# NilFoundation/crypto3-zk

Hardware: AMD Instinct MI355X
Metric: MSM Mpoints/sec, BLS12-381 G1 Pippenger, 2^20 points per GPU (higher is better)
Workload: dtype u32; 1 GPU; BLS12-381 G1 Pippenger MSM, ONE MSM of 1 x 2^20 random points/scalars, bases resident; points_per_gpu=1048576, parallelism=point-range partition x1 + one all-gather of the 144-B partial sums

## Files before the change

### __graft_entry__.py

```python
import importlib.util
import os
import subprocess
import sys

ROOT = os.path.dirname(os.path.abspath(__file__))


def _load_pkg():
    if "crypto3_zk_amd" in sys.modules:
        return sys.modules["crypto3_zk_amd"]
    pkg_dir = os.path.join(ROOT, "crypto3-zk_amd")
    spec = importlib.util.spec_from_file_location("crypto3_zk_amd", os.path.join(pkg_dir, "__init__.py"),
                                                  submodule_search_locations=[pkg_dir])
    mod = importlib.util.module_from_spec(spec)
    sys.modules["crypto3_zk_amd"] = mod
    spec.loader.exec_module(mod)
    return mod


def build() -> None:
    env = dict(os.environ)
    subprocess.check_call(["make", "-C", os.path.join(ROOT, "crypto3-zk_amd"), "-j4", "all"], env=env)
    subprocess.check_call(["make", "-C", os.path.join(ROOT, "oracle"), "liboracle.so"], env=env)
    subprocess.check_call(["make", "-j2", "-C", os.path.join(ROOT, "tests", "cpp")], env=env)
    subprocess.check_call(["make", "-C", os.path.join(ROOT, "tests", "cpp"), "-f", "merkle.mk"], env=env)
    subprocess.check_call(["make", "-C", os.path.join(ROOT, "tests", "cpp"), "-f", "pow.mk"], env=env)
    subprocess.check_call(["make", "-j2", "-C", os.path.join(ROOT, "tests", "cpp"), "-f", "pasta.mk"], env=env)
    subprocess.check_call(["make", "-C", os.path.join(ROOT, "tests", "cpp"), "-f", "ipa.mk"], env=env)
    zk = _load_pkg()
    zk.load_library()


def smoke() -> None:
    import numpy as np

    sys.path.insert(0, os.path.join(ROOT, "oracle"))
    import cport as cp
    import pyoracle as po

    zk = _load_pkg()
    ctx = zk.Context(0)
    n = 5000
    ks = cp.random_fr(0, 1, n)
    bases = ctx.bases_from_scalars(zk.BLS12_381, zk.G1, ks)
    pts, inf = bases.download()
    exp_pts, _ = cp.batch_mul(0, 1, ks)
    assert (pts == exp_pts).all(), "device fixed-base multiples differ from the oracle"
    sc = cp.random_fr(0, 2, n)
    aff, is_inf = ctx.msm_affine(bases, sc)
    exp, einf = cp.msm(0, 1, pts, sc, chunks=2)
    assert is_inf == einf and (aff == exp).all(), "MSM differs from the oracle"
    grp = zk.DeviceGroup([0, 0])
    gb = grp.upload_bases(zk.BLS12_381, zk.G1, pts)
    gaff, ginf = grp.msm_affine(gb, sc)
    assert ginf == einf and (gaff == exp).all(), "device-group MSM differs from the oracle"
    gb.free()
    grp.close()
    k2 = cp.random_fr(0, 4, 300)
    b2 = ctx.bases_from_scalars(zk.BLS12_381, zk.G2, k2)
    p2, _ = b2.download()
    s2 = cp.random_fr(0, 5, 300)
    aff2, inf2 = ctx.msm_affine(b2, s2)
    exp2, einf2 = cp.msm(0, 2, p2, s2, chunks=2)
    assert inf2 == einf2 and (aff2 == exp2).all(), "G2 MSM differs from the oracle"
    b2.free()
    log_m = 12
    w = np.array(po.to_limbs(po.BLS12_381.root_of_unity(log_m), 4), dtype=np.uint64)
    a = cp.random_fr(0, 3, 2 << log_m).reshape(2, 1 << log_m, 4)
    got = ctx.ntt(zk.BLS12_381, a, log_m, w)
    assert (got == cp.ntt(0, a, log_m, w)).all(), "NTT differs from the oracle"
    assert (ctx.ntt(zk.BLS12_381, got, log_m, w, inverse=True) == a).all()
    bases.free()
    M, nin = 1024, 10
    g16 = cp.Groth16(0, M, nin, seed=3)
    kind, m = cp.domain_choice(M + nin + 1, 32)
    wd = np.array(po.to_limbs(po.BLS12_381.root_of_unity((M + nin).bit_length()), 4), dtype=np.uint64)
    gen = np.array(po.to_limbs(po.BLS12_381.fr_generator, 4), dtype=np.uint64)
    g16.set_domain(kind, m, wd)
    r1cs = ctx.upload_r1cs(zk.BLS12_381, g16.M, g16.n, g16.N, g16.csr(0), g16.csr(1), g16.csr(2))
    assert (r1cs.kind, r1cs.m) == (kind, m) == (2, 1040), "the constraint system's domain is not the reference's choice"
    z = np.concatenate([np.array([[1, 0, 0, 0]], dtype=np.uint64), g16.assignment()])
    assert (ctx.groth16_witness_h(r1cs, z, wd, gen) == g16.witness_map(wd, gen)).all(), "witness map over the step domain differs from the oracle"
    r1cs.free()
    import hashlib
    state = hashlib.sha256(b"zkhip smoke").digest()
    k = next(k for k in range(1 << 20)
             if int.from_bytes(hashlib.sha256(hashlib.sha256(state + (12345 + k).to_bytes(4, "big")).digest()).digest()[28:], "big") & 0xFFF == 0)
    assert ctx.pow_grind(state, 12345, 0xFFF) == (12345 + k, k + 1), "the device's proof of work is not the first accepted nonce"
    ctx.close()
    print("smoke ok: G1 MSM n=5000 (one context and a device group of two), G2 MSM n=300, NTT 2^12 x 2 and the witness map over a step radix-2 domain bit-exact against the oracle; proof of work (12 bits) = the reference loop's nonce")


if __name__ == "__main__":
    build()
    if len(sys.argv) > 1 and sys.argv[1] == "smoke":
        smoke()
```

### crypto3-zk_amd/csrc/ctx.hpp

```cpp
#pragma once
#include <hip/hip_runtime.h>

#include <algorithm>
#include <cassert>
#include <cstdint>
#include <cstdio>
#include <cstring>
#include <map>
#include <memory>
#include <mutex>
#include <string>
#include <type_traits>
#include <unordered_map>
#include <unordered_set>
#include <utility>
#include <vector>

#include "../../include/zkhip.h"
#include "options.hpp"
#include "table_cache.hpp"
#include "zk_defs.hpp"

#define ZK_HIP_CHECK(ctx, expr)                                                                  \
    do {                                                                                         \
        hipError_t e__ = (expr);                                                                 \
        if (e__ != hipSuccess) {                                                                 \
            (ctx)->last_error = std::string(#expr) + ": " + hipGetErrorString(e__);              \
            return e__ == hipErrorOutOfMemory ? ZKHIP_ERR_OOM : ZKHIP_ERR_HIP;                   \
        }                                                                                        \
    } while (0)

#define ZK_TRY(expr)              \
    do {                          \
        int rc__ = (expr);        \
        if (rc__ != 0) return rc__; \
    } while (0)

inline bool zk_curve_known(int curve) { return curve >= zkhip::CURVE_BLS12_381 && curve <= zkhip::CURVE_VESTA; }
inline bool zk_curve_pairing(int curve) { return curve == zkhip::CURVE_BLS12_381 || curve == zkhip::CURVE_BN254; }
inline bool zk_group_known(int group) { return group == zkhip::GROUP_G1 || group == zkhip::GROUP_G2; }
inline bool zk_curve_group_known(int curve, int group) { return zk_curve_known(curve) && (group == zkhip::GROUP_G1 || (group == zkhip::GROUP_G2 && zk_curve_pairing(curve))); }
#define ZK_ARGS(ctx, curve) if (!(ctx) || !zk_curve_known(curve)) return ZKHIP_ERR_INVALID
#define ZK_ARGS_PAIRING(ctx, curve) if (!(ctx) || !zk_curve_pairing(curve)) return ZKHIP_ERR_INVALID
#define ZK_ENTER(ctx) ZK_HIP_CHECK(ctx, hipSetDevice((ctx)->device))
inline bool zk_any_null(const void *const *p, size_t count) {
    return std::any_of(p, p + count, [](const void *q) { return !q; });
}

inline dim3 grid_1d(size_t count, unsigned threads = 256) {
    const size_t groups = (count + threads - 1) / threads;
    assert(groups < ((size_t)1 << 31));
    return dim3((unsigned)groups);
}

static constexpr int ZK_MSM_MAX_C = 21;

enum : uint32_t { ZK_STATUS_GATHER_RANGE = 1u, ZK_STATUS_MSM_PLAN_OVERFLOW = 2u, ZK_STATUS_LOOKUP_NOT_IN_TABLE = 4u, ZK_STATUS_LOOKUP_SORT_OVERFLOW = 8u };

struct zkhip_ctx;

struct DevBuf {
    uint32_t *p = nullptr;
    DevBuf() = default;
    DevBuf(const DevBuf &) = delete;
    DevBuf &operator=(const DevBuf &) = delete;
    DevBuf(DevBuf &&o) noexcept : p(o.p) { o.p = nullptr; }
    DevBuf &operator=(DevBuf &&o) noexcept {
        if (this != &o) {
            reset();
            p = o.p;
            o.p = nullptr;
        }
        return *this;
    }
    ~DevBuf() { reset(); }
    void reset() {
        if (p) (void)hipFree(p);
        p = nullptr;
    }
    int alloc(zkhip_ctx *ctx, size_t bytes);
    operator uint32_t *() const { return p; }
    template <class T>
    T *as() const { return reinterpret_cast<T *>(p); }
};
template <bool Pinned = false>
struct GrowBuf {
    void *p = nullptr;
    size_t cap = 0;
    GrowBuf() = default;
    GrowBuf(const GrowBuf &) = delete;
    GrowBuf &operator=(const GrowBuf &) = delete;
    GrowBuf(GrowBuf &&o) noexcept : p(o.p), cap(o.cap) { o.p = nullptr, o.cap = 0; }
    ~GrowBuf() { reset(); }
    void reset() {
        if (p) (void)(Pinned ? hipHostFree(p) : hipFree(p));
        p = nullptr;
        cap = 0;
    }
    int reserve(zkhip_ctx *ctx, size_t bytes, size_t slack = 0);
    template <class T>
    T *as() const { return static_cast<T *>(p); }
};
struct ZkHipDelete {
    void operator()(hipEvent_t e) const { (void)hipEventDestroy(e); }
    void operator()(hipStream_t s) const { (void)hipStreamDestroy(s); }
    void operator()(hipGraphExec_t g) const { (void)hipGraphExecDestroy(g); }
};
using EventOwner = std::unique_ptr<std::remove_pointer_t<hipEvent_t>, ZkHipDelete>;
using StreamOwner = std::unique_ptr<std::remove_pointer_t<hipStream_t>, ZkHipDelete>;
using GraphExecOwner = std::unique_ptr<std::remove_pointer_t<hipGraphExec_t>, ZkHipDelete>;
inline hipError_t zk_event_create(EventOwner &e, unsigned flags = hipEventDefault) {
    hipEvent_t raw = nullptr;
    const hipError_t rc = hipEventCreateWithFlags(&raw, flags);
    e.reset(raw);
    return rc;
}

struct zkhip_bases {
    int curve, group;
    size_t n;
    size_t stride_u32;
    DevBuf d;
    int c_tab = 0, ntab = 1;
    int win_rank = 0, win_world = 1;
    int nslots = 1;
    bool tables() const { return c_tab > 0; }
    int local_windows() const { return win_rank < ntab ? (ntab - win_rank + win_world - 1) / win_world : 0; }
    int slot_of_local(int lw) const { return lw + (win_rank != 0 ? 1 : 0); }
};

struct ZkEventPair {
    EventOwner a, b;
};

struct ZkProfile {
    bool on = false;
    bool last_recorded = false;
    std::string filter;
    std::vector<std::pair<std::string, ZkEventPair>> pending;
    std::vector<ZkEventPair> pool;
    std::map<std::string, std::pair<double, uint64_t>> acc;
};

static constexpr int NTT_MAX_PASSES = 32;
struct NttTables {
    int curve;
    size_t log_m;
    int inverse;
    bool has_coset;
    int smax, tile_log;
    uint64_t omega[4], coset[4];
    int lo_bits;
    DevBuf d_tw[NTT_MAX_PASSES];
    DevBuf d_stage[NTT_MAX_PASSES];
    DevBuf d_prepost;
    DevBuf d_lo, d_hi;
    DevBuf d_clo, d_chi;
    DevBuf d_scale;
    DevBuf d_base;
};
struct NttExtTables {
    int curve;
    size_t log_m, log_k;
    uint64_t omega_big[4];
    DevBuf d_pre;
};
struct DomTables {
    int curve, kind;
    size_t m, n0, n1;
    uint64_t omega[4], shift[4], coset[4];
    bool has_coset;
    DevBuf d_T;
    DevBuf d_Tinv;
    DevBuf d_consts;
    DevBuf d_zinv;
    size_t nz = 1;
    uint64_t w0[4], w1[4];
    uint64_t coset1[4];
};

struct ZkGraph {
    GraphExecOwner exec;
    uint64_t ws_epoch = 0;
    DevBuf d_ptrs;
};

struct zkhip_ctx {
    int device = 0;
    hipStream_t stream = nullptr;
    StreamOwner own_stream;
    EventOwner order_event;
    std::string last_error;
    std::multimap<size_t, void *> alloc_free;
    std::unordered_map<void *, size_t> alloc_live;
    size_t alloc_cached_bytes = 0, opt_alloc_cache_bytes = (size_t)16 << 30;
    std::mutex alloc_mutex;
    DevBuf d_status;
    GrowBuf<> ws;
    size_t ws_off = 0, ws_floor = 0;
    std::unordered_set<const void *> lds_configured;
    std::unordered_map<std::string, ZkGraph> graphs;
    std::unordered_map<std::string, int> graph_seen;
    uint64_t ws_epoch = 0;
    bool capturing = false;
    void *batch_dptrs_override = nullptr;
    int opt_msm_graphs = 0;
    GrowBuf<> msm_host_buf;
    int opt_msm_window_bits = 0;
    int opt_msm_sets = 0;
    int opt_msm_sort_tile_log = 14;
    int opt_ec_ntt_table_lanes = 0;
    int opt_msm_share_sort = 1;
    int opt_msm_tail_quads = 1;
    int opt_msm_tail_fold = 16;
    int opt_msm_tail_fold_g2 = 1;
    int opt_msm_fold_run = 0;
    int opt_msm_segment_log = -1;
    int opt_ntt_radix_log = 8;
    int opt_ntt_tile_log = 3;
    int opt_poly_coset_extend = 1;
    int opt_ntt_pair = 1;
    int opt_msm_precompute = 1;
    int opt_msm_shard_rank = 0, opt_msm_shard_world = 1;
    int opt_stream_priority = 0;
    int opt_msm_precompute_min = 32;
    ZkProfile prof;
    TableCache<NttTables> ntt_tables{24};
    TableCache<NttExtTables> ntt_ext_tables{16};
    TableCache<DomTables> dom_tables{8};
    GrowBuf<> dom_ws;

    zkhip_ctx() = default;
    ~zkhip_ctx();

    int ws_reserve(size_t bytes) {
        if (bytes <= ws.cap) return 0;
        if (capturing) {
            last_error = "workspace growth during graph capture";
            return ZKHIP_ERR_HIP;
        }
        ++ws_epoch;
        return ws.reserve(this, bytes, (bytes >> 3) + (1 << 20));
    }
    void ws_reset() { ws_off = ws_floor; }
    static size_t ws_round(size_t bytes) { return (bytes + 255) & ~(size_t)255; }
    int stream_drain() {
        ZK_HIP_CHECK(this, hipStreamSynchronize(stream));
        return 0;
    }

    void prof_begin(const char *name) {
        prof.last_recorded = false;
        if (!prof.on) return;
        if (!prof.filter.empty() && strncmp(name, prof.filter.c_str(), prof.filter.size()) != 0) return;
        prof.last_recorded = true;
        ZkEventPair ev;
        if (!prof.pool.empty()) {
            ev = std::move(prof.pool.back());
            prof.pool.pop_back();
        } else {
            (void)zk_event_create(ev.a);
            (void)zk_event_create(ev.b);
        }
        (void)hipEventRecord(ev.a.get(), stream);
        prof.pending.emplace_back(name, std::move(ev));
    }
    void prof_end() {
        if (!prof.on || !prof.last_recorded) return;
        (void)hipEventRecord(prof.pending.back().second.b.get(), stream);
    }
    void prof_collect() {
        if (prof.pending.empty()) return;
        (void)hipStreamSynchronize(stream);
        for (auto &p : prof.pending) {
            float ms = 0;
            (void)hipEventElapsedTime(&ms, p.second.a.get(), p.second.b.get());
            auto &a = prof.acc[p.first];
            a.first += ms;
            a.second += 1;
            prof.pool.push_back(std::move(p.second));
        }
        prof.pending.clear();
    }
};

inline int DevBuf::alloc(zkhip_ctx *ctx, size_t bytes) {
    reset();
    const hipError_t e = hipMalloc((void **)&p, bytes);
    if (e == hipSuccess) return 0;
    (void)hipGetLastError();
    ctx->last_error = "hipMalloc(" + std::to_string(bytes) + " bytes): " + hipGetErrorString(e);
    return ZKHIP_ERR_OOM;
}
template <bool Pinned>
int GrowBuf<Pinned>::reserve(zkhip_ctx *ctx, size_t bytes, size_t slack) {
    if (bytes <= cap) return 0;
    if (p) ZK_HIP_CHECK(ctx, hipStreamSynchronize(ctx->stream));
    reset();
    const hipError_t e = Pinned ? hipHostMalloc(&p, bytes + slack, hipHostMallocPortable) : hipMalloc(&p, bytes + slack);
    if (e != hipSuccess) {
        (void)hipGetLastError();
        p = nullptr;
        ctx->last_error = std::string(Pinned ? "hipHostMalloc(" : "hipMalloc(") + std::to_string(bytes + slack) + " bytes): " + hipGetErrorString(e);
        return ZKHIP_ERR_OOM;
    }
    cap = bytes + slack;
    return 0;
}

struct WsCount {
    size_t bytes = 0;
    template <class T>
    void take(T *&, size_t count) { bytes += zkhip_ctx::ws_round(count * sizeof(T)); }
};
struct WsBump {
    zkhip_ctx *ctx;
    template <class T>
    void take(T *&p, size_t count) {
        p = reinterpret_cast<T *>(ctx->ws.as<char>() + ctx->ws_off);
        ctx->ws_off += zkhip_ctx::ws_round(count * sizeof(T));
    }
};
template <class T>
struct WsOne {
    size_t count;
    T *p;
    template <class Arena>
    void layout(Arena &a) { a.take(p, count); }
};
template <class Layout>
size_t ws_bytes(Layout &l) {
    WsCount a;
    l.layout(a);
    return a.bytes;
}
template <class Layout>
int ws_place(zkhip_ctx *ctx, Layout &l, size_t above = 0) {
    const size_t end = ctx->ws_floor + ws_bytes(l);
    ZK_TRY(ctx->ws_reserve(end + above));
    ctx->ws_reset();
    WsBump a{ctx};
    l.layout(a);
    if (ctx->ws_off > end || end + above > ctx->ws.cap) {
        ctx->last_error = "workspace layout took " + std::to_string(ctx->ws_off - ctx->ws_floor) + " bytes of " + std::to_string(end - ctx->ws_floor) + " reserved";
        return ZKHIP_ERR_RANGE;
    }
    return 0;
}

inline int ws_upload(zkhip_ctx *ctx, void *d_dst, const void *src, size_t bytes) {
    if (ctx->capturing) {
        ctx->last_error = "host table upload during graph capture";
        return ZKHIP_ERR_HIP;
    }
    ZK_HIP_CHECK(ctx, hipMemcpyAsync(d_dst, src, bytes, hipMemcpyHostToDevice, ctx->stream));
    return 0;
}

#define ZK_MAX_LDS(ctx, kernel, bytes)                                                                                              \
    do {                                                                                                                            \
        const void *fn__ = reinterpret_cast<const void *>(&kernel);                                                                 \
        if ((ctx)->lds_configured.insert(fn__).second)                                                                              \
            ZK_HIP_CHECK(ctx, hipFuncSetAttribute(fn__, hipFuncAttributeMaxDynamicSharedMemorySize, (int)(bytes)));                 \
    } while (0)

#define ZK_LAUNCH(ctx, name, kernel, grid, block, lds, ...)                        \
    do {                                                                           \
        (ctx)->prof_begin(name);                                                   \
        hipLaunchKernelGGL(kernel, grid, block, lds, (ctx)->stream, __VA_ARGS__);  \
        (ctx)->prof_end();                                                         \
        ZK_HIP_CHECK(ctx, hipGetLastError());                                      \
    } while (0)

int zk_msm_run(zkhip_ctx *ctx, const zkhip_bases *bases, size_t offset, size_t n, const uint32_t *d_scalars, uint32_t *d_out_jac);
int zk_msm_run_batch(zkhip_ctx *ctx, size_t count, const zkhip_bases *const *bases, const size_t *offsets, const size_t *ns,
                     const uint32_t *const *d_scalars, uint32_t *const *d_outs);
size_t zk_coord_limbs64(int curve, int group);
int zk_bases_to_mont(zkhip_ctx *ctx, zkhip_bases *b, const uint32_t *d_canonical, const uint8_t *d_inf);
size_t zk_point_words(int curve, int group);
int zk_msm_auto_window(size_t n);
int zk_scalar_bits(int curve);
int zk_bases_decompress(zkhip_ctx *ctx, zkhip_bases *b, const uint8_t *d_octets, uint32_t *d_err);
void zk_graphs_clear(zkhip_ctx *ctx);
int zk_bases_precompute(zkhip_ctx *ctx, zkhip_bases *b);
int zk_bases_from_mont(zkhip_ctx *ctx, const zkhip_bases *b, size_t offset, size_t n, uint32_t *d_out, uint8_t *d_inf);
int zk_bases_mul(zkhip_ctx *ctx, zkhip_bases *b, const uint32_t *d_base_canonical , const uint32_t *d_scalars);
int zk_jac_sum(zkhip_ctx *ctx, int curve, int group, const uint32_t *d_pts, size_t count, uint32_t *d_out);
int zk_jac_to_affine(zkhip_ctx *ctx, int curve, int group, const uint32_t *d_jac, uint32_t *d_aff, uint8_t *d_inf);
int zk_ntt_run(zkhip_ctx *ctx, int curve, uint32_t *d_data, size_t log_m, size_t batch, const uint64_t *omega, int inverse,
               const uint64_t *coset);
int zk_ntt_extend(zkhip_ctx *ctx, int curve, uint32_t *d_coeffs, size_t log_m, size_t batch, const uint64_t *omega, uint32_t *d_out, size_t log_k,
                  const uint64_t *omega_big);
int zk_msm_host_reserve(zkhip_ctx *ctx, size_t n);
```

### crypto3-zk_amd/csrc/hosttest.hip

```cpp
#include <cstring>
#include <vector>

#define ZK_NOINLINE_MUL 1
#include "arith_ops.h"
#include "msm_recode.hpp"
#include "pow.hpp"
#include "sha256.hpp"

using namespace zkhip;
using namespace zkhip::arith;

#define FIELD_SWITCH(field, ...)                             \
    switch (field) {                                         \
        case 0: { typedef bls_fq F; __VA_ARGS__; } break;    \
        case 1: { typedef bls_fr F; __VA_ARGS__; } break;    \
        case 2: { typedef bn_fq F; __VA_ARGS__; } break;     \
        case 3: { typedef bn_fr F; __VA_ARGS__; } break;     \
        case 4: { typedef bls_fq2 F; __VA_ARGS__; } break;   \
        case 5: { typedef bn_fq2 F; __VA_ARGS__; } break;    \
        case 6: { typedef bls_fqu F; __VA_ARGS__; } break;   \
        case 7: { typedef bn_fqu F; __VA_ARGS__; } break;    \
        case 8: { typedef bls_fru F; __VA_ARGS__; } break;   \
        case 9: { typedef bn_fru F; __VA_ARGS__; } break;    \
        case 10: { typedef bls_fqu2 F; __VA_ARGS__; } break; \
        case 11: { typedef bn_fqu2 F; __VA_ARGS__; } break;  \
        case 12: { typedef pallas_fq F; __VA_ARGS__; } break; \
        case 13: { typedef pallas_fr F; __VA_ARGS__; } break; \
        case 14: { typedef vesta_fq F; __VA_ARGS__; } break;  \
        case 15: { typedef vesta_fr F; __VA_ARGS__; } break;  \
        case 16: { typedef pallas_fqu F; __VA_ARGS__; } break; \
        case 17: { typedef vesta_fqu F; __VA_ARGS__; } break; \
        case 18: { typedef pallas_fru F; __VA_ARGS__; } break; \
        case 19: { typedef vesta_fru F; __VA_ARGS__; } break; \
        default: return -1;                                  \
    }

extern "C" {

int zkt_field_op(int field, int op, const uint32_t *a, const uint32_t *b, uint32_t *out) {
    if (!field_op_valid(op)) return -1;
    FIELD_SWITCH(field, field_op<F>(op, a, b, out); return 0);
    return -1;
}

int zkt_fu_raw(int type, int op, size_t n, const uint32_t *a, const uint32_t *b, const uint32_t *c, const uint32_t *d, uint32_t *out) {
#define FU_RAW(U)                                                                                                       \
    {                                                                                                                   \
        if (!fu_raw_valid<U>(op)) return -1;                                                                            \
        for (size_t i = 0; i < n; ++i) fu_raw_one<U>(op, a + i * U::L, b + i * U::L, c + i * U::L, d + i * U::L, out + i * U::L); \
        return 0;                                                                                                       \
    }
    switch (type) {
        case 6: FU_RAW(BlsFqU)
        case 7: FU_RAW(BnFqU)
        case 8: FU_RAW(BlsFrU)
        case 9: FU_RAW(BnFrU)
        case 16: FU_RAW(PallasFqU)
        case 17: FU_RAW(VestaFqU)
        case 18: FU_RAW(PallasFrU)
        case 19: FU_RAW(VestaFrU)
        default: return -1;
    }
#undef FU_RAW
}

int zkt_point_chain(int field, const uint32_t *pts, const uint8_t *inf, const uint8_t *neg, size_t n, int mode, uint32_t k,
                    uint32_t *out, uint8_t *out_inf) {
    if (field == 1 || field == 3 || field == 8 || field == 9 || field == 13 || field == 15 || field == 18 || field == 19) return -1;
    FIELD_SWITCH(field, point_chain<F>(pts, inf, neg, n, mode, k, out, out_inf); return 0);
    return -1;
}

static int recode_windows(const uint32_t *scalar, MsmWindows win, int32_t *digits) {
    uint32_t carry = 0;
    for (int w = 0; w < win.W; ++w) {
        uint32_t d = msm_recode(scalar, win.off(w), win.width(w), carry);
        if (d == DIG_NONE) digits[w] = 0;
        else {
            int32_t mag = (int32_t)(d & 0x7FFFFFFFu) + 1;
            digits[w] = (d >> 31) ? -mag : mag;
        }
    }
    return (int)carry;
}

int zkt_recode(const uint32_t *scalar, int c, int W, int32_t *digits) { return recode_windows(scalar, msm_make_windows(c * W, W), digits); }

int zkt_recode_folded(int curve, const uint32_t *scalar, int c, int32_t *digits) {
    uint32_t s[8];
    bool flip = false;
    if (fr_sat_dispatch(curve, [&](auto fr) -> int {
            flip = msm_fold_scalar<typename decltype(fr)::type>(scalar, s);
            return 0;
        }) != 0)
        return -1;
    const int tb = curve == CURVE_BN254 ? 254 : 255, W = msm_windows(tb, c);
    if (recode_windows(s, msm_make_windows(tb, W), digits) != 0) return -1;
    if (flip)
        for (int w = 0; w < W; ++w) digits[w] = -digits[w];
    return W;
}

int zkt_sha256_elements(const uint64_t *elems, size_t n, uint8_t *digest) {
    if (!elems || !digest || n == 0) return -1;
    sha256::hash_elements(elems, n, digest);
    return 0;
}

int zkt_merkle_tree(const uint64_t *leaves, size_t n_leaves, size_t per_leaf, uint8_t *digests) {
    if (!leaves || !digests || n_leaves == 0 || (n_leaves & (n_leaves - 1)) || per_leaf == 0) return -1;
    for (size_t x = 0; x < n_leaves; ++x) sha256::hash_elements(leaves + 4 * x * per_leaf, per_leaf, digests + 32 * x);
    uint8_t *level = digests;
    for (size_t n = n_leaves / 2; n >= 1; n /= 2) {
        uint8_t *up = level + 64 * n;
        for (size_t j = 0; j < n; ++j) sha256::hash_node(level + 64 * j, level + 64 * j + 32, up + 32 * j);
        level = up;
    }
    return 0;
}

uint32_t zkt_pow_candidate(const uint8_t *state, uint32_t nonce) { return pow::candidate(pow::prepare(state), nonce); }

int zkt_pow_grind_cpu(const uint8_t *state, uint32_t start, uint32_t mask, uint64_t max_tries, uint32_t *nonce, uint64_t *tried) {
    if (!state || !nonce || !tried || max_tries > ((uint64_t)1 << 32)) return -1;
    const uint64_t total = max_tries ? max_tries : (uint64_t)1 << 32, k = pow::first_hit(pow::prepare(state), start, mask, total);
    *tried = k < total ? k + 1 : total;
    if (k == total) return 1;
    *nonce = start + (uint32_t)k;
    return 0;
}

int zkt_sha256_bytes(const uint8_t *msg, size_t len, uint8_t *digest) {
    if (!digest || (!msg && len)) return -1;
    pow::hash_bytes(msg, len, digest);
    return 0;
}

}
```

### crypto3-zk_amd/csrc/msm_core.hpp

```cpp
#pragma once
#include <algorithm>
#include <string>
#include <type_traits>
#include <vector>

#ifndef ZK_NOINLINE_MUL2
#define ZK_NOINLINE_MUL2 1
#endif
#include "ctx.hpp"
#include "curve.hpp"
#include "msm_ops.hpp"
#include "msm_recode.hpp"
#include "msm_bucket_acc.hpp"
#include "fu_pair.hpp"
#include "fu_quad.hpp"

namespace {

using namespace zkhip;

constexpr uint32_t MSM_LARGE_BUCKET = 128;
constexpr uint32_t MSM_LARGE_CHUNK = 4096;
#ifndef MSM_G1_THREADS
#define MSM_G1_THREADS 64
#endif
#ifndef MSM_G2_THREADS
#define MSM_G2_THREADS 256
#endif
#ifndef MSM_G2_WAVES
#define MSM_G2_WAVES 2
#endif

template <uint32_t THREADS>
ZK_D void block_inclusive_scan(uint32_t *scratch) {
    const uint32_t t = threadIdx.x;
    __syncthreads();
    for (uint32_t d = 1; d < THREADS; d <<= 1) {
        uint32_t x = t >= d ? scratch[t - d] : 0;
        __syncthreads();
        scratch[t] += x;
        __syncthreads();
    }
}

__global__ __launch_bounds__(256) void msm_scan_local(const uint32_t *__restrict__ hist, uint32_t count, uint32_t *__restrict__ offs,
                                                      uint32_t *__restrict__ block_sums) {
    __shared__ uint32_t part[256];
    const uint32_t t = threadIdx.x, base = blockIdx.x * 1024 + t * 4;
    uint32_t v[4], s = 0;
#pragma unroll
    for (int k = 0; k < 4; ++k) {
        v[k] = base + k < count ? hist[base + k] : 0;
        s += v[k];
    }
    part[t] = s;
    block_inclusive_scan<256>(part);
    uint32_t run = part[t] - s;
#pragma unroll
    for (int k = 0; k < 4; ++k) {
        if (base + k < count) offs[base + k] = run;
        run += v[k];
    }
    if (t == 255) block_sums[blockIdx.x] = part[255];
}

__global__ __launch_bounds__(1024) void msm_scan_top(uint32_t *__restrict__ block_sums, uint32_t nblocks, uint32_t *__restrict__ total) {
    __shared__ uint32_t part[1024];
    const uint32_t t = threadIdx.x;
    const uint32_t per = (nblocks + 1023) / 1024;
    const uint32_t lo = min(nblocks, t * per), hi = min(nblocks, lo + per);
    uint32_t s = 0;
    for (uint32_t i = lo; i < hi; ++i) s += block_sums[i];
    part[t] = s;
    block_inclusive_scan<1024>(part);
    uint32_t run = part[t] - s;
    for (uint32_t i = lo; i < hi; ++i) {
        uint32_t x = block_sums[i];
        block_sums[i] = run;
        run += x;
    }
    if (t == 1023) *total = part[1023];
}

__global__ __launch_bounds__(256) void msm_scan_add(uint32_t *__restrict__ offs, uint32_t count, const uint32_t *__restrict__ block_sums,
                                                    uint32_t *__restrict__ cursor) {
    const uint32_t base = blockIdx.x * 1024 + threadIdx.x * 4;
    const uint32_t add = block_sums[blockIdx.x];
#pragma unroll
    for (int k = 0; k < 4; ++k) {
        if (base + k < count) {
            uint32_t x = offs[base + k] + add;
            offs[base + k] = x;
            cursor[base + k] = x;
        }
    }
}

__global__ __launch_bounds__(1024) void msm_scan_single(const uint32_t *__restrict__ hist, uint32_t count, uint32_t *__restrict__ offs,
                                                        uint32_t *__restrict__ cursor) {
    __shared__ uint32_t part[1024];
    __shared__ uint32_t carry;
    const uint32_t t = threadIdx.x;
    if (t == 0) carry = 0;
    __syncthreads();
    for (uint32_t base = 0; base < count; base += 1024) {
        const uint32_t v = base + t < count ? hist[base + t] : 0;
        part[t] = v;
        block_inclusive_scan<1024>(part);
        const uint32_t excl = carry + part[t] - v;
        if (base + t < count) {
            offs[base + t] = excl;
            if (cursor != offs) cursor[base + t] = excl;
        }
        __syncthreads();
        if (t == 1023) carry += part[1023];
        __syncthreads();
    }
    if (t == 0) offs[count] = carry;
}
constexpr uint32_t MSM_SCAN_SINGLE_MAX = 1u << 16;

inline int msm_scan(zkhip_ctx *ctx, const char *name, const uint32_t *hist, uint32_t count, uint32_t *offs, uint32_t *bsums) {
    if (count <= MSM_SCAN_SINGLE_MAX) {
        ZK_LAUNCH(ctx, name, msm_scan_single, dim3(1), dim3(1024), 0, hist, count, offs, offs);
        return 0;
    }
    const uint32_t nblk = (count + 1023) / 1024;
    ZK_LAUNCH(ctx, name, msm_scan_local, dim3(nblk), dim3(256), 0, hist, count, offs, bsums);
    ZK_LAUNCH(ctx, name, msm_scan_top, dim3(1), dim3(1024), 0, bsums, nblk, offs + count);
    ZK_LAUNCH(ctx, name, msm_scan_add, dim3(nblk), dim3(256), 0, offs, count, bsums, offs);
    return 0;
}

template <class FR>
__global__ __launch_bounds__(256) void msm_digits_only(const uint32_t *__restrict__ scalars, uint32_t n, MsmWindows win, uint32_t wrank,
                                                       uint32_t wworld, uint32_t *__restrict__ dig) {
    uint32_t i = blockIdx.x * blockDim.x + threadIdx.x;
    if (i >= n) return;
    uint32_t s[8];
    const uint32_t flip = msm_fold_scalar<FR>(scalars + (size_t)i * 8, s) ? 0x80000000u : 0u;
    uint32_t carry = 0, next = wrank, lw = 0;
    for (int w = 0; w < win.W; ++w) {
        uint32_t d = msm_recode(s, win.off(w), win.width(w), carry);
        if ((uint32_t)w != next) continue;
        dig[(size_t)lw * n + i] = d == DIG_NONE ? d : d ^ flip;
        next += wworld;
        ++lw;
    }
}

struct SortGeom {
    uint32_t n;
    uint32_t W;
    uint32_t B;
    uint32_t S;
    uint32_t lowb;
    uint32_t nsuper;
    uint32_t tile;
    uint32_t ntile;
    uint32_t slot0;
    uint32_t tables;
    uint32_t bases_n;
    uint32_t base_off;
};
struct SortBig {
    static constexpr uint32_t TILE = 16384, THREADS = 1024;
};
struct SortSmall {
    static constexpr uint32_t TILE = 4096, THREADS = 256;
};
constexpr uint32_t SORT_MAX_LOW = 10;
constexpr uint32_t SORT_MAX_SUPER = 1024;

ZK_D uint32_t sort_key(const SortGeom &g, uint32_t w, uint32_t d) { return (w % g.S) * g.B + (d & 0x7FFFFFFFu); }
ZK_D uint32_t sort_entry(const SortGeom &g, uint32_t w, uint32_t i, uint32_t d) {
    return ((g.tables ? (g.slot0 + w) * g.bases_n : 0u) + g.base_off + i) | (d & 0x80000000u);
}

template <class SZ>
__global__ __launch_bounds__(SZ::THREADS) void msm_sort_hist(const uint32_t *__restrict__ dig, SortGeom g, uint32_t *__restrict__ bh) {
    constexpr uint32_t SORT_TILE = SZ::TILE, SORT_THREADS = SZ::THREADS;
    extern __shared__ uint32_t lh[];
    const uint32_t tile = blockIdx.x, w = blockIdx.y, t = threadIdx.x;
    for (uint32_t k = t; k < g.nsuper; k += SORT_THREADS) lh[k] = 0;
    __syncthreads();
    const uint32_t lo = tile * SORT_TILE, hi = min(g.n, lo + SORT_TILE);
    for (uint32_t i = lo + t; i < hi; i += SORT_THREADS) {
        uint32_t d = dig[(size_t)w * g.n + i];
        if (d != DIG_NONE) atomicAdd(&lh[sort_key(g, w, d) >> g.lowb], 1u);
    }
    __syncthreads();
    const size_t col = (size_t)w * g.ntile + tile, stride = (size_t)g.W * g.ntile;
    for (uint32_t k = t; k < g.nsuper; k += SORT_THREADS) bh[(size_t)k * stride + col] = lh[k];
}

template <uint32_t SORT_THREADS>
ZK_D uint32_t block_excl_scan(uint32_t *v, uint32_t count, uint32_t *scratch ) {
    const uint32_t t = threadIdx.x, per = (count + SORT_THREADS - 1) / SORT_THREADS;
    const uint32_t lo = min(count, t * per), hi = min(count, lo + per);
    uint32_t s = 0;
    for (uint32_t k = lo; k < hi; ++k) s += v[k];
    scratch[t] = s;
    block_inclusive_scan<SORT_THREADS>(scratch);
    const uint32_t total = scratch[SORT_THREADS - 1];
    uint32_t run = scratch[t] - s;
    for (uint32_t k = lo; k < hi; ++k) {
        uint32_t x = v[k];
        v[k] = run;
        run += x;
    }
    __syncthreads();
    return total;
}

template <class SZ>
__global__ __launch_bounds__(SZ::THREADS) void msm_sort_split(const uint32_t *__restrict__ dig, SortGeom g, const uint32_t *__restrict__ bo,
                                                              uint32_t *__restrict__ tmp_idx, uint16_t *__restrict__ tmp_key) {
    constexpr uint32_t SORT_TILE = SZ::TILE, SORT_THREADS = SZ::THREADS;
    extern __shared__ uint32_t sm[];
    uint32_t *loff = sm;
    uint32_t *cur = loff + g.nsuper + 1;
    uint32_t *gbase = cur + g.nsuper;
    uint32_t *scratch = gbase + g.nsuper;
    uint32_t *sidx = scratch + SORT_THREADS;
    uint32_t *skey = sidx + SORT_TILE;
    const uint32_t tile = blockIdx.x, w = blockIdx.y, t = threadIdx.x;
    const size_t col = (size_t)w * g.ntile + tile, stride = (size_t)g.W * g.ntile;
    for (uint32_t k = t; k < g.nsuper; k += SORT_THREADS) {
        loff[k] = 0;
        gbase[k] = bo[(size_t)k * stride + col];
    }
    __syncthreads();
    const uint32_t lo = tile * SORT_TILE, hi = min(g.n, lo + SORT_TILE);
    for (uint32_t i = lo + t; i < hi; i += SORT_THREADS) {
        uint32_t d = dig[(size_t)w * g.n + i];
        if (d != DIG_NONE) atomicAdd(&loff[sort_key(g, w, d) >> g.lowb], 1u);
    }
    __syncthreads();
    const uint32_t total = block_excl_scan<SORT_THREADS>(loff, g.nsuper, scratch);
    if (t == 0) loff[g.nsuper] = total;
    for (uint32_t k = t; k < g.nsuper; k += SORT_THREADS) cur[k] = loff[k];
    __syncthreads();
    for (uint32_t i = lo + t; i < hi; i += SORT_THREADS) {
        uint32_t d = dig[(size_t)w * g.n + i];
        if (d == DIG_NONE) continue;
        const uint32_t key = sort_key(g, w, d);
        const uint32_t r = atomicAdd(&cur[key >> g.lowb], 1u);
        sidx[r] = sort_entry(g, w, i, d);
        skey[r] = key;
    }
    __syncthreads();
    const uint32_t lmask = (1u << g.lowb) - 1;
    for (uint32_t s = t; s < total; s += SORT_THREADS) {
        const uint32_t key = skey[s], bin = key >> g.lowb, pos = gbase[bin] + (s - loff[bin]);
        tmp_idx[pos] = sidx[s];
        tmp_key[pos] = (uint16_t)(key & lmask);
    }
}

constexpr uint32_t SORT_NLOW_MAX = 1u << SORT_MAX_LOW;

template <uint32_t THREADS>
ZK_D void block_scan_counts(const uint32_t *cnt, uint32_t *excl, uint32_t *scratch) {
    constexpr uint32_t CPT = SORT_NLOW_MAX / THREADS;
    const uint32_t t = threadIdx.x;
    uint32_t s = 0;
#pragma unroll
    for (uint32_t k = 0; k < CPT; ++k) s += cnt[t * CPT + k];
    scratch[t] = s;
    block_inclusive_scan<THREADS>(scratch);
    uint32_t run = scratch[t] - s;
#pragma unroll
    for (uint32_t k = 0; k < CPT; ++k) {
        excl[t * CPT + k] = run;
        run += cnt[t * CPT + k];
    }
    __syncthreads();
}

template <class SZ>
__global__ __launch_bounds__(SZ::THREADS) void msm_sort_final(const uint32_t *__restrict__ tmp_idx, const uint16_t *__restrict__ tmp_key, SortGeom g,
                                                              uint32_t nb, const uint32_t *__restrict__ bo, uint32_t *__restrict__ offs,
                                                              uint32_t *__restrict__ idx) {
    constexpr uint32_t SORT_TILE = SZ::TILE, SORT_THREADS = SZ::THREADS;
    __shared__ uint32_t cnt[SORT_NLOW_MAX], cursor[SORT_NLOW_MAX], loff[SORT_NLOW_MAX], cur[SORT_NLOW_MAX], scratch[SORT_THREADS];
    extern __shared__ uint32_t sm[];
    uint32_t *sidx = sm;
    uint16_t *skey = reinterpret_cast<uint16_t *>(sidx + SORT_TILE);
    const uint32_t grp = blockIdx.x, t = threadIdx.x;
    const size_t stride = (size_t)g.W * g.ntile;
    const uint32_t start = bo[(size_t)grp * stride];
    const uint32_t end = bo[(size_t)(grp + 1) * stride];
    const uint32_t nlow = 1u << g.lowb;
    for (uint32_t k = t; k < SORT_NLOW_MAX; k += SORT_THREADS) cnt[k] = 0;
    __syncthreads();
    for (uint32_t k = start + t; k < end; k += SORT_THREADS) atomicAdd(&cnt[tmp_key[k]], 1u);
    __syncthreads();
    block_scan_counts<SORT_THREADS>(cnt, cursor, scratch);
    for (uint32_t k = t; k < nlow; k += SORT_THREADS) {
        const uint32_t bucket = grp * nlow + k;
        cursor[k] += start;
        if (bucket < nb) offs[bucket] = cursor[k];
    }
    if (grp + 1 == g.nsuper && t == 0) offs[nb] = end;
    __syncthreads();
    for (uint32_t c0 = start; c0 < end; c0 += SORT_TILE) {
        const uint32_t c1 = min(end, c0 + SORT_TILE);
        for (uint32_t k = t; k < SORT_NLOW_MAX; k += SORT_THREADS) cnt[k] = 0;
        __syncthreads();
        for (uint32_t k = c0 + t; k < c1; k += SORT_THREADS) atomicAdd(&cnt[tmp_key[k]], 1u);
        __syncthreads();
        block_scan_counts<SORT_THREADS>(cnt, loff, scratch);
        for (uint32_t k = t; k < SORT_NLOW_MAX; k += SORT_THREADS) cur[k] = loff[k];
        __syncthreads();
        for (uint32_t k = c0 + t; k < c1; k += SORT_THREADS) {
            const uint32_t key = tmp_key[k];
            const uint32_t r = atomicAdd(&cur[key], 1u);
            sidx[r] = tmp_idx[k];
            skey[r] = (uint16_t)key;
        }
        __syncthreads();
        for (uint32_t s = t; s < c1 - c0; s += SORT_THREADS) {
            const uint32_t key = skey[s];
            idx[cursor[key] + (s - loff[key])] = sidx[s];
        }
        __syncthreads();
        for (uint32_t k = t; k < SORT_NLOW_MAX; k += SORT_THREADS) cursor[k] += cnt[k];
        __syncthreads();
    }
}

constexpr uint32_t SIZE_BINS = MSM_LARGE_BUCKET + 2;

ZK_D uint32_t size_bin(uint32_t size, uint32_t large) {
    if (size == 0 || size > large) return SIZE_BINS - 1;
    return size > MSM_LARGE_BUCKET ? 0 : 1 + MSM_LARGE_BUCKET - size;
}

__global__ __launch_bounds__(256) void msm_size_hist(const uint32_t *__restrict__ offs, uint32_t nbuckets, uint32_t nblocks,
                                                     uint32_t large, uint32_t *__restrict__ bh) {
    __shared__ uint32_t lh[SIZE_BINS];
    const uint32_t t = threadIdx.x;
    if (t < SIZE_BINS) lh[t] = 0;
    __syncthreads();
    for (uint32_t g = blockIdx.x * 1024 + t; g < min(nbuckets, (blockIdx.x + 1) * 1024); g += 256)
        atomicAdd(&lh[size_bin(offs[g + 1] - offs[g], large)], 1u);
    __syncthreads();
    if (t < SIZE_BINS) bh[(size_t)t * nblocks + blockIdx.x] = lh[t];
}

__global__ __launch_bounds__(256) void msm_size_scatter(const uint32_t *__restrict__ offs, uint32_t nbuckets, uint32_t nblocks,
                                                        uint32_t large, const uint32_t *__restrict__ bo, uint32_t *__restrict__ order) {
    __shared__ uint32_t cur[SIZE_BINS];
    const uint32_t t = threadIdx.x;
    if (t < SIZE_BINS) cur[t] = bo[(size_t)t * nblocks + blockIdx.x];
    __syncthreads();
    for (uint32_t g = blockIdx.x * 1024 + t; g < min(nbuckets, (blockIdx.x + 1) * 1024); g += 256)
        order[atomicAdd(&cur[size_bin(offs[g + 1] - offs[g], large)], 1u)] = g;
}

__global__ __launch_bounds__(256) void msm_plan_large(const uint32_t *__restrict__ offs, uint32_t nbuckets, uint32_t *__restrict__ plan,
                                                      uint32_t *__restrict__ tasks, uint32_t *__restrict__ large, uint32_t task_cap,
                                                      uint32_t large_cap, uint32_t thresh, uint32_t *__restrict__ status) {
    uint32_t g = blockIdx.x * blockDim.x + threadIdx.x;
    if (g >= nbuckets) return;
    uint32_t lo = offs[g], hi = offs[g + 1], size = hi - lo;
    if (size <= thresh) return;
    uint32_t nt = (size + MSM_LARGE_CHUNK - 1) / MSM_LARGE_CHUNK;
    uint32_t first = atomicAdd(&plan[0], nt);
    uint32_t slot = atomicAdd(&plan[1], 1u);
    if (first + nt > task_cap || slot >= large_cap) {
        atomicOr(status, ZK_STATUS_MSM_PLAN_OVERFLOW);
        return;
    }
    for (uint32_t t = 0; t < nt; ++t) {
        tasks[3 * (first + t)] = g;
        tasks[3 * (first + t) + 1] = lo + t * MSM_LARGE_CHUNK;
        tasks[3 * (first + t) + 2] = min(hi, lo + (t + 1) * MSM_LARGE_CHUNK);
    }
    large[3 * slot] = g;
    large[3 * slot + 1] = first;
    large[3 * slot + 2] = nt;
}

template <class F, int LPB>
__global__ __launch_bounds__(128) void msm_bucket_large(const uint32_t *__restrict__ bases, const uint32_t *__restrict__ idx,
                                                        const uint32_t *__restrict__ plan, const uint32_t *__restrict__ tasks,
                                                        uint32_t *__restrict__ partials) {
    constexpr int NL = FieldOps<F>::WORDS;
    extern __shared__ __attribute__((aligned(16))) uint32_t lds[];
    const uint32_t ntasks = plan[0];
    for (uint32_t task = blockIdx.x; task < ntasks; task += gridDim.x) {
        const uint32_t lo = tasks[3 * task + 1], hi = tasks[3 * task + 2], t = threadIdx.x / LPB;
        XYZZ<F> acc = XYZZ<F>::infinity();
        for (uint32_t k = lo + t; k < hi; k += blockDim.x / LPB) {
            uint32_t e = idx[k];
            Affine<F> p = affine_load<F>(bases + (size_t)(e & 0x7FFFFFFFu) * (2 * NL));
            acc = xyzz_madd(acc, p, (e >> 31) != 0);
        }
        xyzz_store<F>(lds + (size_t)t * (4 * NL), acc);
        __syncthreads();
        for (uint32_t d = blockDim.x / LPB / 2; d >= 1; d >>= 1) {
            if (t < d) {
                acc = xyzz_add(xyzz_load<F>(lds + (size_t)t * (4 * NL)), xyzz_load<F>(lds + (size_t)(t + d) * (4 * NL)));
                xyzz_store<F>(lds + (size_t)t * (4 * NL), acc);
            }
            __syncthreads();
        }
        if (t == 0) xyzz_store<F>(partials + (size_t)task * (4 * NL), acc);
        __syncthreads();
    }
}

template <class F, int LPB>
__global__ __launch_bounds__(64) void msm_large_combine(const uint32_t *__restrict__ plan, const uint32_t *__restrict__ large,
                                                        const uint32_t *__restrict__ partials, uint32_t *__restrict__ buckets) {
    constexpr int NL = FieldOps<F>::WORDS;
    extern __shared__ __attribute__((aligned(16))) uint32_t lds[];
    const uint32_t nlarge = plan[1], t = threadIdx.x / LPB;
    for (uint32_t j = blockIdx.x; j < nlarge; j += gridDim.x) {
        const uint32_t g = large[3 * j], first = large[3 * j + 1], nt = large[3 * j + 2];
        XYZZ<F> acc = XYZZ<F>::infinity();
        for (uint32_t k = t; k < nt; k += 64 / LPB) acc = xyzz_add(acc, xyzz_load<F>(partials + (size_t)(first + k) * (4 * NL)));
        if (nt > 1) {
            xyzz_store<F>(lds + (size_t)t * (4 * NL), acc);
            __syncthreads();
            for (uint32_t d = 32 / LPB; d >= 1; d >>= 1) {
                if (t < d && t + d < nt) {
                    acc = xyzz_add(xyzz_load<F>(lds + (size_t)t * (4 * NL)), xyzz_load<F>(lds + (size_t)(t + d) * (4 * NL)));
                    xyzz_store<F>(lds + (size_t)t * (4 * NL), acc);
                }
                __syncthreads();
            }
        }
        if (t == 0) xyzz_store<F>(buckets + (size_t)g * (4 * NL), acc);
        __syncthreads();
    }
}

template <class F, int LPB>
__global__ __launch_bounds__(256) void msm_bucket_merge(uint32_t *__restrict__ buckets, uint32_t B, uint32_t q, uint32_t cur) {
    constexpr int NL = FieldOps<F>::WORDS;
    uint32_t g = (blockIdx.x * blockDim.x + threadIdx.x) / LPB;
    if (g >= q * B) return;
    const uint32_t s = g / B;
    uint32_t *dst = buckets + (size_t)g * (4 * NL);
    XYZZ<F> acc = xyzz_load<F>(dst);
    for (uint32_t k = 1; k < 4; ++k)
        if (s + k * q < cur) acc = xyzz_add(acc, xyzz_load<F>(buckets + ((size_t)g + (size_t)k * q * B) * (4 * NL)));
    xyzz_store<F>(dst, acc);
}

constexpr int MSM_TAIL_THREADS = 256;

template <class F>
ZK_D XYZZ<F> block_tree_sum(uint32_t *lds, XYZZ<F> acc, uint32_t t, uint32_t nthreads) {
    constexpr int NL = FieldOps<F>::WORDS;
    xyzz_store<F>(lds + (size_t)t * (4 * NL), acc);
    __syncthreads();
    for (uint32_t d = nthreads / 2; d >= 1; d >>= 1) {
        if (t < d) {
            acc = xyzz_add(xyzz_load<F>(lds + (size_t)t * (4 * NL)), xyzz_load<F>(lds + (size_t)(t + d) * (4 * NL)));
            xyzz_store<F>(lds + (size_t)t * (4 * NL), acc);
        }
        __syncthreads();
    }
    return acc;
}

template <class F, int LPB>
#ifndef ZK_TAIL_WAVES
#define ZK_TAIL_WAVES 2
#endif
__global__ __launch_bounds__(MSM_TAIL_THREADS, ZK_TAIL_WAVES) void msm_bucket_red(const uint32_t *__restrict__ buckets, uint32_t B, uint32_t L, uint32_t nseg,
                                                                   uint32_t nblk, uint32_t *__restrict__ partial) {
    constexpr int NL = FieldOps<F>::WORDS;
    extern __shared__ __attribute__((aligned(16))) uint32_t lds[];
    constexpr uint32_t SLOTS = MSM_TAIL_THREADS / LPB;
    const uint32_t t = threadIdx.x / LPB, w = blockIdx.x / nblk, seg = (blockIdx.x % nblk) * SLOTS + t;
    XYZZ<F> sum = XYZZ<F>::infinity();
    if (seg < nseg) {
        const uint32_t *base = buckets + ((size_t)w * B + (size_t)seg * L) * (4 * NL);
        if (L == 1) {
            sum = xyzz_mul_small(xyzz_load<F>(base), seg + 1);
        } else {
            XYZZ<F> run = XYZZ<F>::infinity();
            for (int b = (int)L - 1; b >= 0; --b) {
                run = xyzz_add(run, xyzz_load<F>(base + (size_t)b * (4 * NL)));
                sum = xyzz_add(sum, run);
            }
            if (seg != 0) sum = xyzz_add(sum, xyzz_mul_small(run, seg * L));
        }
    }
    sum = block_tree_sum<F>(lds, sum, t, SLOTS);
    if (t == 0) xyzz_store<F>(partial + (size_t)blockIdx.x * (4 * NL), sum);
}

template <class F, int LPB>
__global__ __launch_bounds__(256) void msm_window_sum(const uint32_t *__restrict__ partial, uint32_t nblk, uint32_t *__restrict__ winsum) {
    constexpr int NL = FieldOps<F>::WORDS;
    extern __shared__ __attribute__((aligned(16))) uint32_t lds[];
    const uint32_t w = blockIdx.x, t = threadIdx.x / LPB, slots = blockDim.x / LPB;
    XYZZ<F> acc = XYZZ<F>::infinity();
    for (uint32_t j = t; j < nblk; j += slots) acc = xyzz_add(acc, xyzz_load<F>(partial + ((size_t)w * nblk + j) * (4 * NL)));
    if (nblk > 1) acc = block_tree_sum<F>(lds, acc, t, slots);
    if (t == 0) xyzz_store<F>(winsum + (size_t)w * (4 * NL), acc);
}
inline uint32_t msm_window_threads(uint32_t nblk, int lanes_per_point) { return (size_t)nblk * lanes_per_point > 128 ? 256u : 64u; }

struct MsmFold {
    uint32_t B, C, R, log_c;
    uint32_t run;
    uint32_t m_row, m_col;
};
inline MsmFold msm_fold_geom(const zkhip_ctx *ctx, uint32_t B) {
    MsmFold g;
    int lb = 0;
    while ((1u << lb) < B) ++lb;
    g.B = B;
    g.log_c = (uint32_t)((lb + 1) / 2);
    g.C = 1u << g.log_c;
    g.R = B >> g.log_c;
    g.run = ctx->opt_msm_fold_run > 0 ? (uint32_t)ctx->opt_msm_fold_run : (B >= (1u << 18) ? 8u : 4u);
    g.run = std::max(1u, std::min(g.run, g.R));
    g.m_row = g.C / g.run;
    g.m_col = g.R / g.run;
    return g;
}

template <class FA, int LA, class FT, int LT>
__global__ __launch_bounds__(MSM_TAIL_THREADS, ZK_TAIL_WAVES) void msm_fold(const uint32_t *__restrict__ buckets, MsmFold g, uint32_t *__restrict__ level2) {
    constexpr int NL = FieldOps<FA>::WORDS;
    constexpr uint32_t SA = MSM_TAIL_THREADS / LA, ST = MSM_TAIL_THREADS / LT, PW = 4 * NL;
    extern __shared__ __attribute__((aligned(16))) uint32_t lds[];
    const uint32_t half_wgs = g.B / (SA * g.run);
    const uint32_t w = blockIdx.x / (2 * half_wgs), k = blockIdx.x % (2 * half_wgs);
    const bool col = k >= half_wgs;
    const uint32_t wg = col ? k - half_wgs : k, s = threadIdx.x / LA;
    const uint32_t m = col ? g.m_col : g.m_row, G = SA / m;
    uint32_t first, stride, slot;
    if (!col) {
        first = (wg * G + s / m) * g.C + s % m;
        stride = m;
        slot = s;
    } else {
        const uint32_t j = s / G, ll = s % G;
        first = j * g.C + wg * G + ll;
        stride = m * g.C;
        slot = ll * m + j;
    }
    {
        const uint32_t *src = buckets + ((size_t)w * g.B + first) * PW;
        XYZZ<FA> acc = xyzz_load<FA>(src);
        for (uint32_t i = 1; i < g.run; ++i) acc = xyzz_add(acc, xyzz_load<FA>(src + (size_t)i * stride * PW));
        xyzz_store<FA>(lds + (size_t)slot * PW, acc);
    }
    __syncthreads();
    const uint32_t t = threadIdx.x / LT;
    for (uint32_t half = m / 2; half >= 1; half >>= 1) {
        const uint32_t adds = G * half;
        for (uint32_t idx = t; idx < adds; idx += ST) {
            uint32_t *p = lds + (size_t)((idx / half) * m + idx % half) * PW;
            xyzz_store<FT>(p, xyzz_add(xyzz_load<FT>(p), xyzz_load<FT>(p + (size_t)half * PW)));
        }
        __syncthreads();
    }
    for (uint32_t i = t; i < G; i += ST) {
        const uint32_t o = wg * G + i;
        if (col || o != 0)
            xyzz_store<FT>(level2 + (((size_t)2 * w + (col ? 0 : 1)) * g.C + (col ? o : o - 1)) * PW, xyzz_load<FT>(lds + (size_t)i * m * PW));
    }
}

template <class F>
ZK_D void xyzz_store_canonical_jacobian(uint32_t *dst, const XYZZ<F> &p) {
    constexpr int CW = FieldOps<F>::CANON_WORDS;
    Jacobian<F> j = xyzz_to_jacobian(p);
    FieldOps<F>::to_canonical(dst, j.X);
    FieldOps<F>::to_canonical(dst + CW, j.Y);
    FieldOps<F>::to_canonical(dst + 2 * CW, j.Z);
}

template <class F, int LPB>
__global__ __launch_bounds__(64) void msm_final_fold(const uint32_t *__restrict__ winsum, uint32_t count, uint32_t shift, uint32_t *const *__restrict__ outs,
                                                     uint32_t *__restrict__ out) {
    constexpr int NL = FieldOps<F>::WORDS;
    if (blockIdx.x >= count || threadIdx.x >= LPB) return;
    XYZZ<F> acc = xyzz_load<F>(winsum + ((size_t)2 * blockIdx.x + 1) * (4 * NL));
    if (!acc.is_inf())
        for (uint32_t i = 0; i < shift; ++i) acc = xyzz_dbl(acc);
    acc = xyzz_add(acc, xyzz_load<F>(winsum + (size_t)2 * blockIdx.x * (4 * NL)));
    xyzz_store_canonical_jacobian<F>(outs ? outs[blockIdx.x] : out, acc);
}

template <class F, int LPB>
__global__ __launch_bounds__(64) void msm_final(const uint32_t *__restrict__ winsum, int W, MsmWindows win, uint32_t *__restrict__ out_jac) {
    constexpr int NL = FieldOps<F>::WORDS;
    if (blockIdx.x != 0 || threadIdx.x >= LPB) return;
    XYZZ<F> acc = XYZZ<F>::infinity();
    for (int w = W - 1; w >= 0; --w) {
        if (!acc.is_inf())
            for (int i = 0; i < win.width(w); ++i) acc = xyzz_dbl(acc);
        acc = xyzz_add(acc, xyzz_load<F>(winsum + (size_t)w * (4 * NL)));
    }
    xyzz_store_canonical_jacobian<F>(out_jac, acc);
}

template <class F>
__global__ __launch_bounds__(256) void bases_to_mont(const uint32_t *__restrict__ canon, const uint8_t *__restrict__ inf, uint32_t n,
                                                     uint32_t *__restrict__ pts) {
    typedef FieldOps<F> O;
    uint32_t i = blockIdx.x * blockDim.x + threadIdx.x;
    if (i >= n) return;
    const uint32_t *c = canon + (size_t)i * (2 * O::CANON_WORDS);
    Affine<F> a;
    if (inf != nullptr && inf[i]) a = Affine<F>::infinity();
    else a = {O::from_canonical(c), O::from_canonical(c + O::CANON_WORDS)};
    affine_store<F>(pts + (size_t)i * (2 * O::WORDS), a);
}

template <class F>
__global__ __launch_bounds__(256) void bases_from_mont(const uint32_t *__restrict__ pts, uint32_t n, uint32_t *__restrict__ out,
                                                       uint8_t *__restrict__ inf) {
    typedef FieldOps<F> O;
    uint32_t i = blockIdx.x * blockDim.x + threadIdx.x;
    if (i >= n) return;
    Affine<F> a = affine_load<F>(pts + (size_t)i * (2 * O::WORDS));
    inf[i] = a.is_inf() ? 1 : 0;
    uint32_t *o = out + (size_t)i * (2 * O::CANON_WORDS);
    O::to_canonical(o, a.x);
    O::to_canonical(o + O::CANON_WORDS, a.y);
}

template <class F>
__global__ __launch_bounds__(64) void bases_mul(uint32_t *__restrict__ pts, const uint32_t *__restrict__ base_canonical,
                                                const uint32_t *__restrict__ scalars, uint32_t n) {
    constexpr int NL = FieldOps<F>::WORDS;
    uint32_t i = blockIdx.x * blockDim.x + threadIdx.x;
    if (i >= n) return;
    Affine<F> g = {FieldOps<F>::from_canonical(base_canonical), FieldOps<F>::from_canonical(base_canonical + FieldOps<F>::CANON_WORDS)};
    const uint32_t *s = scalars + (size_t)i * 8;
    XYZZ<F> acc = XYZZ<F>::infinity();
    for (int b = 255; b >= 0; --b) {
        acc = xyzz_dbl(acc);
        if ((s[b >> 5] >> (b & 31)) & 1) acc = xyzz_madd(acc, g);
    }
    affine_store<F>(pts + (size_t)i * (2 * NL), xyzz_to_affine(acc));
}

constexpr int FIXED_WBITS = 8, FIXED_NW = 32, FIXED_ROW = 1 << FIXED_WBITS;
template <class F>
__global__ __launch_bounds__(64) void bases_fixed_table(const uint32_t *__restrict__ base_canonical, uint32_t *__restrict__ tab, uint32_t *__restrict__ tmp) {
    typedef FieldOps<F> O;
    constexpr int NL = O::WORDS;
    const uint32_t w = blockIdx.x * blockDim.x + threadIdx.x;
    if (w >= FIXED_NW) return;
    Affine<F> g = {O::from_canonical(base_canonical), O::from_canonical(base_canonical + O::CANON_WORDS)};
    XYZZ<F> P = XYZZ<F>::from_affine(g);
    for (uint32_t k = 0; k < w * FIXED_WBITS; ++k) P = xyzz_dbl(P);
    uint32_t *mine = tmp + (size_t)w * FIXED_ROW * (5 * NL);
    XYZZ<F> acc = P;
    F pre = F::one();
    for (uint32_t d = 1; d < FIXED_ROW; ++d) {
        if (d > 1) acc = xyzz_add(acc, P);
        uint32_t *slot = mine + (size_t)d * (5 * NL);
        xyzz_store<F>(slot, acc);
        pre = O::mul(pre, O::mul(acc.ZZ, acc.ZZZ));
        O::store(slot + 4 * NL, pre);
    }
    F inv = O::inv(pre);
    for (uint32_t d = FIXED_ROW; d-- > 1;) {
        const uint32_t *slot = mine + (size_t)d * (5 * NL);
        XYZZ<F> q = xyzz_load<F>(slot);
        F before = d > 1 ? O::load(mine + (size_t)(d - 1) * (5 * NL) + 4 * NL) : F::one();
        F dinv = O::mul(inv, before);
        inv = O::mul(inv, O::mul(q.ZZ, q.ZZZ));
        Affine<F> a = {O::mul(q.X, O::mul(dinv, q.ZZZ)), O::mul(q.Y, O::mul(dinv, q.ZZ))};
        affine_store<F>(tab + ((size_t)w * FIXED_ROW + d) * (2 * NL), a);
    }
}
constexpr uint32_t FIXED_CHUNK = 8;
template <class F>
__global__ __launch_bounds__(64) void bases_mul_fixed(uint32_t *__restrict__ pts, const uint32_t *__restrict__ tab, const uint32_t *__restrict__ scalars,
                                                      uint32_t n, uint32_t *__restrict__ tmp) {
    typedef FieldOps<F> O;
    constexpr int NL = O::WORDS;
    const uint32_t lo = (blockIdx.x * blockDim.x + threadIdx.x) * FIXED_CHUNK;
    if (lo >= n) return;
    const uint32_t cnt = n - lo < FIXED_CHUNK ? n - lo : FIXED_CHUNK;
    F pre = F::one();
    for (uint32_t k = 0; k < cnt; ++k) {
        const uint32_t *s = scalars + (size_t)(lo + k) * 8;
        XYZZ<F> acc = XYZZ<F>::infinity();
        for (uint32_t w = 0; w < FIXED_NW; ++w) {
            const uint32_t d = (s[w >> 2] >> ((w & 3) * 8)) & 0xFFu;
            if (d) acc = xyzz_madd(acc, affine_load<F>(tab + ((size_t)w * FIXED_ROW + d) * (2 * NL)));
        }
        uint32_t *slot = tmp + (size_t)(lo + k) * (5 * NL);
        xyzz_store<F>(slot, acc);
        if (!acc.is_inf()) pre = O::mul(pre, O::mul(acc.ZZ, acc.ZZZ));
        O::store(slot + 4 * NL, pre);
    }
    F inv = O::inv(pre);
    for (uint32_t k = cnt; k-- > 0;) {
        const uint32_t *slot = tmp + (size_t)(lo + k) * (5 * NL);
        XYZZ<F> q = xyzz_load<F>(slot);
        if (q.is_inf()) {
            affine_store<F>(pts + (size_t)(lo + k) * (2 * NL), Affine<F>::infinity());
            continue;
        }
        F before = k > 0 ? O::load(tmp + (size_t)(lo + k - 1) * (5 * NL) + 4 * NL) : F::one();
        F dinv = O::mul(inv, before);
        inv = O::mul(inv, O::mul(q.ZZ, q.ZZZ));
        Affine<F> a = {O::mul(q.X, O::mul(dinv, q.ZZZ)), O::mul(q.Y, O::mul(dinv, q.ZZ))};
        affine_store<F>(pts + (size_t)(lo + k) * (2 * NL), a);
    }
}

template <class F>
__global__ __launch_bounds__(64) void bases_precompute_range(uint32_t *__restrict__ pts, uint32_t n, uint32_t lo, uint32_t cnt, MsmWindows win,
                                                             uint32_t wrank, uint32_t wworld, uint32_t *__restrict__ tmp) {
    const int W = win.W;
    typedef FieldOps<F> O;
    constexpr int NL = O::WORDS;
    uint32_t j = blockIdx.x * blockDim.x + threadIdx.x;
    if (j >= cnt) return;
    const uint32_t i = lo + j;
    const uint32_t extra = wrank != 0 ? 1u : 0u;
    auto slot_ptr = [&](uint32_t w) { return pts + ((size_t)(w / wworld + extra) * n + i) * (2 * NL); };
    Affine<F> p = affine_load<F>(pts + (size_t)i * (2 * NL));
    if (p.is_inf()) {
        for (uint32_t w = (wrank != 0 ? wrank : wworld); w < (uint32_t)W; w += wworld) affine_store<F>(slot_ptr(w), Affine<F>::infinity());
        return;
    }
    XYZZ<F> acc = XYZZ<F>::from_affine(p);
    F pre = F::one();
    uint32_t kept = 0;
    for (int w = 1; w < W; ++w) {
        for (int k = 0; k < win.width(w - 1); ++k) acc = xyzz_dbl(acc);
        if ((uint32_t)w % wworld != wrank) continue;
        uint32_t *slot = tmp + ((size_t)kept * cnt + j) * (5 * NL);
        xyzz_store<F>(slot, acc);
        pre = O::mul(pre, O::mul(acc.ZZ, acc.ZZZ));
        O::store(slot + 4 * NL, pre);
        ++kept;
    }
    if (kept == 0) return;
    F inv = O::inv(pre);
    uint32_t w = ((uint32_t)(W - 1) - wrank) / wworld * wworld + wrank;
    for (uint32_t k = kept; k-- > 0; w -= wworld) {
        const uint32_t *slot = tmp + ((size_t)k * cnt + j) * (5 * NL);
        XYZZ<F> q = xyzz_load<F>(slot);
        F before = k > 0 ? O::load(tmp + ((size_t)(k - 1) * cnt + j) * (5 * NL) + 4 * NL) : F::one();
        F dinv = O::mul(inv, before);
        inv = O::mul(inv, O::mul(q.ZZ, q.ZZZ));
        Affine<F> a = {O::mul(q.X, O::mul(dinv, q.ZZZ)), O::mul(q.Y, O::mul(dinv, q.ZZ))};
        affine_store<F>(slot_ptr(w), a);
    }
}

template <class F>
__global__ void jac_to_affine_k(const uint32_t *__restrict__ jac, uint32_t *__restrict__ aff, uint8_t *__restrict__ inf) {
    typedef FieldOps<F> O;
    constexpr int CW = O::CANON_WORDS;
    if (blockIdx.x != 0 || threadIdx.x != 0) return;
    Jacobian<F> j = {O::from_canonical(jac), O::from_canonical(jac + CW), O::from_canonical(jac + 2 * CW)};
    XYZZ<F> q = xyzz_from_jacobian(j);
    inf[0] = q.is_inf() ? 1 : 0;
    Affine<F> a = xyzz_to_affine(q);
    O::to_canonical(aff, a.x);
    O::to_canonical(aff + CW, a.y);
}

template <class F>
__global__ void jac_sum_k(const uint32_t *__restrict__ jac, uint32_t count, uint32_t *__restrict__ out) {
    typedef FieldOps<F> O;
    constexpr int CW = O::CANON_WORDS;
    if (blockIdx.x != 0 || threadIdx.x != 0) return;
    XYZZ<F> acc = XYZZ<F>::infinity();
    for (uint32_t i = 0; i < count; ++i) {
        const uint32_t *p = jac + (size_t)i * 3 * CW;
        Jacobian<F> j = {O::from_canonical(p), O::from_canonical(p + CW), O::from_canonical(p + 2 * CW)};
        acc = xyzz_add(acc, xyzz_from_jacobian(j));
    }
    Jacobian<F> r = xyzz_to_jacobian(acc);
    O::to_canonical(out, r.X);
    O::to_canonical(out + CW, r.Y);
    O::to_canonical(out + 2 * CW, r.Z);
}

template <class F>
__global__ void msm_write_infinity(uint32_t *out_jac) {
    if (blockIdx.x != 0 || threadIdx.x != 0) return;
    xyzz_store_canonical_jacobian<F>(out_jac, XYZZ<F>::infinity());
}

template <class F, int LPB>
__global__ __launch_bounds__(64) void msm_final_batch(const uint32_t *__restrict__ winsum, uint32_t count, uint32_t *const *__restrict__ outs) {
    constexpr int NL = FieldOps<F>::WORDS;
    constexpr int CW = FieldOps<F>::CANON_WORDS;
    if (blockIdx.x >= count || threadIdx.x >= LPB) return;
    Jacobian<F> j = xyzz_to_jacobian(xyzz_load<F>(winsum + (size_t)blockIdx.x * (4 * NL)));
    uint32_t *out = outs[blockIdx.x];
    FieldOps<F>::to_canonical(out, j.X);
    FieldOps<F>::to_canonical(out + CW, j.Y);
    FieldOps<F>::to_canonical(out + 2 * CW, j.Z);
}


inline uint32_t msm_tail_segment(const zkhip_ctx *ctx, uint32_t B, size_t sets, int lanes_per_point) {
    uint32_t L = 1;
    if (ctx->opt_msm_segment_log >= 0) L = 1u << std::min(ctx->opt_msm_segment_log, 8);
    else {
        const size_t lanes = sets * B * (size_t)lanes_per_point;
        while (L < 16 && lanes / L > 65536) L <<= 1;
        while (L < 64 && lanes / L > 262144) L <<= 1;
    }
    return std::min(B, L);
}

struct MsmTailGeom {
    uint32_t L, nseg;
    uint32_t slots, nblk;
    uint32_t wthreads;
    size_t lds_red, lds_win;
};
template <class Lane>
MsmTailGeom msm_tail_geom(const zkhip_ctx *ctx, uint32_t B, size_t sets) {
    constexpr size_t point_bytes = (size_t)4 * FieldOps<typename Lane::type>::WORDS * 4;
    constexpr int XL = Lane::LANES;
    MsmTailGeom t;
    t.L = msm_tail_segment(ctx, B, sets, XL);
    t.nseg = B / t.L;
    t.slots = MSM_TAIL_THREADS / XL;
    t.nblk = (t.nseg + t.slots - 1) / t.slots;
    t.wthreads = msm_window_threads(t.nblk, XL);
    t.lds_red = t.slots * point_bytes;
    t.lds_win = t.wthreads / XL * point_bytes;
    return t;
}

template <class Lane, class Final>
int msm_tail(zkhip_ctx *ctx, const uint32_t *sets, size_t nsets, uint32_t B, uint32_t *segsum, size_t segsum_blocks, uint32_t *winsum, Final final) {
    typedef typename Lane::type TX;
    constexpr int XL = Lane::LANES;
    const MsmTailGeom t = msm_tail_geom<Lane>(ctx, B, nsets);
    if (nsets * t.nblk > segsum_blocks) {
        ctx->last_error = "MSM tail of " + std::to_string(nsets * t.nblk) + " workgroups over a partial-sum buffer for " + std::to_string(segsum_blocks);
        return ZKHIP_ERR_RANGE;
    }
    ZK_MAX_LDS(ctx, (msm_bucket_red<TX, XL>), t.lds_red);
    ZK_LAUNCH(ctx, "msm_bucket_red", (msm_bucket_red<TX, XL>), dim3((unsigned)(nsets * t.nblk)), dim3(MSM_TAIL_THREADS), t.lds_red, sets, B, t.L, t.nseg, t.nblk,
              segsum);
    ZK_LAUNCH(ctx, "msm_window_sum", (msm_window_sum<TX, XL>), dim3((unsigned)nsets), dim3(t.wthreads), t.lds_win, segsum, t.nblk, winsum);
    return final();
}

template <class F>
bool msm_fold_applies(const zkhip_ctx *ctx, uint32_t B, bool tables) {
    if (FieldOps<F>::WORDS > 16 && !ctx->opt_msm_tail_fold_g2) return false;
    if (!tables || ctx->opt_msm_tail_fold <= 0 || B < (1u << std::min(ctx->opt_msm_tail_fold, 30))) return false;
    const MsmFold g = msm_fold_geom(ctx, B);
    const uint32_t sa = MSM_TAIL_THREADS / BucketLane<F>::LANES;
    return g.m_col >= 1 && g.m_row <= sa && g.m_col <= sa && B >= sa * g.run && g.m_row * g.run == g.C && g.m_col * g.run == g.R;
}
template <class F>
struct MsmFoldBuffers {
    static constexpr size_t PW = (size_t)4 * FieldOps<F>::WORDS;
    MsmFold g{};
    size_t nsets = 0;
    uint32_t *level2 = nullptr, *segsum = nullptr, *winsum = nullptr;
    MsmFoldBuffers() = default;
    MsmFoldBuffers(const zkhip_ctx *ctx, uint32_t B, size_t nsets_) : g(msm_fold_geom(ctx, B)), nsets(nsets_) {}
    size_t level2_words() const { return nsets * 2 * g.C * PW; }
    size_t segsum_blocks() const { return nsets * 2 * ((g.C + 63) / 64); }
    template <class Arena>
    void layout(Arena &a) {
        a.take(level2, level2_words());
        a.take(segsum, segsum_blocks() * PW);
        a.take(winsum, nsets * 2 * PW);
    }
};

template <class F, class Lane>
int msm_fold_tail(zkhip_ctx *ctx, const uint32_t *sets, const MsmFoldBuffers<F> &fb, uint32_t *const *d_outs, uint32_t *d_out) {
    constexpr int NL = FieldOps<F>::WORDS;
    typedef typename BucketLane<F>::type FL;
    constexpr int LPB = BucketLane<F>::LANES;
    typedef typename QuadLane<F>::type TQ;
    constexpr int QL = QuadLane<F>::LANES;
    const MsmFold &g = fb.g;
    const size_t nsets = fb.nsets;
    ZK_HIP_CHECK(ctx, hipMemsetAsync(fb.level2, 0, fb.level2_words() * 4, ctx->stream));
    const size_t lds = (size_t)MSM_TAIL_THREADS / LPB * 4 * NL * 4;
    ZK_MAX_LDS(ctx, (msm_fold<FL, LPB, TQ, QL>), lds);
    ZK_LAUNCH(ctx, "msm_fold", (msm_fold<FL, LPB, TQ, QL>), dim3((unsigned)(nsets * (g.B / (MSM_TAIL_THREADS / LPB * g.run)) * 2)), dim3(MSM_TAIL_THREADS), lds,
              sets, g, fb.level2);
    auto level2 = [&](auto lane) -> int {
        typedef decltype(lane) X;
        return msm_tail<X>(ctx, fb.level2, 2 * nsets, g.C, fb.segsum, fb.segsum_blocks(), fb.winsum, [&]() -> int {
            ZK_LAUNCH(ctx, "msm_final", (msm_final_fold<typename X::type, X::LANES>), dim3((unsigned)nsets), dim3(64), 0, fb.winsum, (uint32_t)nsets, g.log_c, d_outs, d_out);
            return 0;
        });
    };
    if (QuadLane<F>::AVAILABLE && ctx->opt_msm_tail_quads && 2 * nsets * g.C <= ((size_t)1 << 18)) return level2(QuadLane<F>());
    return level2(Lane());
}

struct MsmPlan {
    int c, W_all, W;
    uint32_t B, S, nb;
    MsmWindows win;
    uint32_t wrank, wworld;
    bool tables;
};

inline MsmPlan msm_plan(const zkhip_ctx *ctx, const zkhip_bases *bases, size_t n) {
    MsmPlan p;
    p.tables = bases->tables();
    int c = p.tables ? bases->c_tab : ctx->opt_msm_window_bits;
    if (c <= 0) c = zk_msm_auto_window(n);
    p.c = std::max(2, std::min(ZK_MSM_MAX_C, c));
    if (!p.tables) p.c = std::min(p.c, 16);
    p.W_all = msm_windows(zk_scalar_bits(bases->curve), p.c);
    p.win = msm_make_windows(zk_scalar_bits(bases->curve), p.W_all);
    p.wrank = p.tables ? (uint32_t)bases->win_rank : 0u;
    p.wworld = p.tables ? (uint32_t)bases->win_world : 1u;
    p.W = p.tables ? bases->local_windows() : p.W_all;
    p.B = 1u << (p.c - 1);
    if (!p.tables) p.S = (uint32_t)p.W;
    else {
        int s = ctx->opt_msm_sets;
        if (s <= 0) s = (int)((zk_msm_target_lanes() + p.B - 1) / p.B);
        p.S = (uint32_t)std::max(1, std::min(p.W, s));
        while (p.S > 1 && (uint64_t)p.S * p.B > ((uint64_t)SORT_MAX_SUPER << SORT_MAX_LOW)) --p.S;
    }
    p.nb = p.S * p.B;
    return p;
}

template <class SZ>
int msm_sort_run(zkhip_ctx *ctx, const SortGeom &g, uint32_t nbh, const uint32_t *dig, uint32_t *bh, uint32_t *bo, uint32_t *bsums, uint32_t *tmp_idx,
                 uint16_t *tmp_key, uint32_t *offs, uint32_t *idx) {
    const size_t lds_hist = (size_t)g.nsuper * 4;
    const size_t lds_split = ((size_t)3 * g.nsuper + 1 + SZ::THREADS + 2 * SZ::TILE) * 4;
    const size_t lds_final = (size_t)SZ::TILE * 6;
    if (lds_split > 48 * 1024) ZK_MAX_LDS(ctx, msm_sort_split<SZ>, 160 * 1024 - 256);
    if (lds_final > 40 * 1024) ZK_MAX_LDS(ctx, msm_sort_final<SZ>, 160 * 1024 - (4 * SORT_NLOW_MAX + SZ::THREADS) * 4 - 256);
    ZK_LAUNCH(ctx, "msm_sort_hist", msm_sort_hist<SZ>, dim3(g.ntile, g.W), dim3(SZ::THREADS), lds_hist, dig, g, bh);
    ZK_TRY(msm_scan(ctx, "msm_scan", bh, nbh, bo, bsums));
    ZK_LAUNCH(ctx, "msm_sort_split", msm_sort_split<SZ>, dim3(g.ntile, g.W), dim3(SZ::THREADS), lds_split, dig, g, bo, tmp_idx, tmp_key);
    ZK_LAUNCH(ctx, "msm_sort_final", msm_sort_final<SZ>, dim3(g.nsuper), dim3(SZ::THREADS), lds_final, tmp_idx, tmp_key, g, g.S * g.B, bo, offs, idx);
    return 0;
}

struct MsmCall {
    MsmPlan P;
    SortGeom g;
    bool big_tiles;
    uint32_t nbh;
    uint32_t sblk, nsh;
    int Sr;
    uint32_t segsum_blocks;
    bool fold;
    uint32_t large_thresh, large_cap, task_cap;
    size_t entries() const { return (size_t)P.W * g.n; }
};

template <class F>
int msm_call_plan(const zkhip_ctx *ctx, const zkhip_bases *bases, size_t offset, size_t n, bool batch_member, MsmCall &c, std::string &error) {
    const MsmPlan &P = c.P = msm_plan(ctx, bases, n);
    if ((uint64_t)P.W * n >= (1ull << 32) || (uint64_t)bases->nslots * bases->n >= (1ull << 31)) {
        error = "MSM of " + std::to_string(n) + " points x " + std::to_string(P.W) + " windows exceeds the 32-bit entry index (split the range)";
        return ZKHIP_ERR_RANGE;
    }
    SortGeom &g = c.g;
    g.n = (uint32_t)n;
    g.W = (uint32_t)P.W;
    g.B = P.B;
    g.S = P.S;
    g.lowb = (uint32_t)std::min<int>(SORT_MAX_LOW, P.c - 1);
    g.nsuper = (P.nb + (1u << g.lowb) - 1) >> g.lowb;
    c.big_tiles = ctx->opt_msm_sort_tile_log >= 14;
    g.tile = c.big_tiles ? SortBig::TILE : SortSmall::TILE;
    g.ntile = (uint32_t)((n + g.tile - 1) / g.tile);
    g.tables = P.tables ? 1u : 0u;
    g.slot0 = P.tables ? (uint32_t)bases->slot_of_local(0) : 0u;
    g.bases_n = (uint32_t)bases->n;
    g.base_off = (uint32_t)offset;
    if (g.nsuper > SORT_MAX_SUPER) return ZKHIP_ERR_RANGE;
    const size_t nbh64 = (size_t)g.nsuper * g.W * g.ntile;
    if (nbh64 >= (1ull << 31)) return ZKHIP_ERR_RANGE;
    c.nbh = (uint32_t)nbh64;
    c.sblk = (P.nb + 1023) / 1024;
    c.nsh = SIZE_BINS * c.sblk;
    c.Sr = P.tables ? 1 : P.W;
    c.segsum_blocks = std::max(msm_tail_geom<TailLane<F>>(ctx, P.B, c.Sr).nblk, msm_tail_geom<QuadLane<F>>(ctx, P.B, c.Sr).nblk);
    c.fold = !batch_member && msm_fold_applies<F>(ctx, P.B, P.tables);
    c.large_thresh = (uint32_t)std::max<size_t>(MSM_LARGE_BUCKET, 4 * ((c.entries() + P.nb - 1) / P.nb));
    c.large_cap = (uint32_t)(c.entries() / c.large_thresh + 1);
    c.task_cap = (uint32_t)(c.entries() / MSM_LARGE_CHUNK + c.large_cap + 1);
    return 0;
}

template <class F>
struct MsmBuffers {
    static constexpr size_t PW = (size_t)4 * FieldOps<F>::WORDS;
    const MsmCall &c;
    uint32_t *dig, *bh, *bo, *bsums, *tmp_idx;
    uint16_t *tmp_key;
    uint32_t *offs, *idx, *buckets;
    uint32_t *sh, *so, *ssums, *order;
    uint32_t *segsum, *winsum;
    MsmFoldBuffers<F> fb;
    uint32_t *plan, *tasks, *large, *partials;
    MsmBuffers(const zkhip_ctx *ctx, const MsmCall &call) : c(call) {
        if (c.fold) fb = MsmFoldBuffers<F>(ctx, c.P.B, 1);
    }
    template <class Arena>
    void layout(Arena &a) {
        a.take(dig, c.entries());
        a.take(bh, c.nbh);
        a.take(bo, (size_t)c.nbh + 1);
        a.take(bsums, (c.nbh + 1023) / 1024);
        a.take(tmp_idx, c.entries());
        a.take(tmp_key, c.entries());
        a.take(offs, (size_t)c.P.nb + 1);
        a.take(idx, c.entries());
        a.take(buckets, c.P.nb * PW);
        a.take(sh, (size_t)c.nsh + 1);
        a.take(so, (size_t)c.nsh + 1);
        a.take(ssums, (c.nsh + 1023) / 1024);
        a.take(order, c.P.nb);
        a.take(segsum, (size_t)c.Sr * c.segsum_blocks * PW);
        a.take(winsum, (size_t)std::max(1, c.Sr) * PW);
        if (c.fold) fb.layout(a);
        a.take(plan, 4);
        a.take(tasks, (size_t)c.task_cap * 3);
        a.take(large, (size_t)c.large_cap * 3);
        a.take(partials, c.task_cap * PW);
    }
};

template <class F>
int msm_stages(zkhip_ctx *ctx, const zkhip_bases *bases, const MsmCall &c, const MsmBuffers<F> &w, const uint32_t *d_scalars, bool reuse_sort) {
    constexpr int NL = FieldOps<F>::WORDS;
    typedef typename BucketLane<F>::type FL;
    constexpr int LPB = BucketLane<F>::LANES;
    const MsmPlan &P = c.P;
    const uint32_t n = c.g.n, nb = P.nb;
    const uint32_t *d_b = bases->d;
    if (!reuse_sort) {
        ZK_TRY(fr_sat_dispatch(bases->curve, [&](auto fr) -> int {
            typedef typename decltype(fr)::type FR;
            ZK_LAUNCH(ctx, "msm_digits", msm_digits_only<FR>, grid_1d(n), dim3(256), 0, d_scalars, n, P.win, P.wrank, P.wworld, w.dig);
            return 0;
        }));
        ZK_TRY((c.big_tiles ? msm_sort_run<SortBig> : msm_sort_run<SortSmall>)(ctx, c.g, c.nbh, w.dig, w.bh, w.bo, w.bsums, w.tmp_idx, w.tmp_key, w.offs, w.idx));
        ZK_LAUNCH(ctx, "msm_size_sort", msm_size_hist, dim3(c.sblk), dim3(256), 0, w.offs, nb, c.sblk, c.large_thresh, w.sh);
        ZK_TRY(msm_scan(ctx, "msm_size_sort", w.sh, c.nsh, w.so, w.ssums));
        ZK_LAUNCH(ctx, "msm_size_sort", msm_size_scatter, dim3(c.sblk), dim3(256), 0, w.offs, nb, c.sblk, c.large_thresh, w.so, w.order);
    }
    if constexpr (FieldOps<F>::WORDS <= 16) {
        constexpr int NT = MSM_G1_THREADS;
        size_t lds_acc = LdsAcc<F, NT>::BYTES;
        ZK_MAX_LDS(ctx, (msm_bucket_acc_lds<F, NT, 3>), lds_acc);
        ZK_LAUNCH(ctx, "msm_bucket_acc", (msm_bucket_acc_lds<F, NT, 3>), dim3((nb + NT - 1) / NT), dim3(NT), lds_acc, d_b, w.offs, w.idx, nb, c.large_thresh,
                  w.order, w.buckets);
    } else {
        constexpr int NT = MSM_G2_THREADS, WAVES = MSM_G2_WAVES;
        size_t lds_acc = LdsAcc<FL, NT>::BYTES;
        ZK_MAX_LDS(ctx, (msm_bucket_acc_lds<FL, NT, WAVES, LPB>), lds_acc);
        ZK_LAUNCH(ctx, "msm_bucket_acc", (msm_bucket_acc_lds<FL, NT, WAVES, LPB>), dim3((unsigned)(((size_t)nb * LPB + NT - 1) / NT)), dim3(NT), lds_acc, d_b,
                  w.offs, w.idx, nb, c.large_thresh, w.order, w.buckets);
    }
    if (!reuse_sort) {
        ZK_HIP_CHECK(ctx, hipMemsetAsync(w.plan, 0, 16, ctx->stream));
        ZK_LAUNCH(ctx, "msm_plan_large", msm_plan_large, grid_1d(nb), dim3(256), 0, w.offs, nb, w.plan, w.tasks, w.large, c.task_cap, c.large_cap,
                  c.large_thresh, ctx->d_status);
    }
    {
        size_t lds_large = (size_t)128 / LPB * 4 * NL * 4;
        if (lds_large > 48 * 1024) ZK_MAX_LDS(ctx, (msm_bucket_large<FL, LPB>), lds_large);
        unsigned grid_large = (unsigned)std::min<size_t>(c.task_cap, 512);
        ZK_LAUNCH(ctx, "msm_bucket_large", (msm_bucket_large<FL, LPB>), dim3(grid_large), dim3(128), lds_large, d_b, w.idx, w.plan, w.tasks, w.partials);
        ZK_LAUNCH(ctx, "msm_bucket_large", (msm_large_combine<FL, LPB>), dim3((unsigned)std::min<uint32_t>(c.large_cap, 256)), dim3(64),
                  (size_t)64 / LPB * 4 * NL * 4, w.plan, w.large, w.partials, w.buckets);
    }
    if (P.tables) {
        for (uint32_t cur = P.S; cur > 1;) {
            const uint32_t q = (cur + 3) / 4;
            ZK_LAUNCH(ctx, "msm_bucket_merge", (msm_bucket_merge<FL, LPB>), grid_1d((size_t)q * P.B * LPB), dim3(256), 0, w.buckets, P.B, q,
                      cur);
            cur = q;
        }
    }
    return 0;
}

template <class F>
int msm_run_t(zkhip_ctx *ctx, const zkhip_bases *bases, size_t offset, size_t n, const uint32_t *d_scalars, uint32_t *d_out_jac) {
    MsmCall c;
    ZK_TRY(msm_call_plan<F>(ctx, bases, offset, n, false, c, ctx->last_error));
    MsmBuffers<F> w(ctx, c);
    ZK_TRY(ws_place(ctx, w));
    ZK_TRY(msm_stages<F>(ctx, bases, c, w, d_scalars, false));
    if (c.fold) return msm_fold_tail<F, TailLane<F>>(ctx, w.buckets, w.fb, nullptr, d_out_jac);
    auto tail = [&](auto lane) -> int {
        typedef decltype(lane) X;
        return msm_tail<X>(ctx, w.buckets, (size_t)c.Sr, c.P.B, w.segsum, (size_t)c.Sr * c.segsum_blocks, w.winsum, [&]() -> int {
            ZK_LAUNCH(ctx, "msm_final", (msm_final<typename X::type, X::LANES>), dim3(1), dim3(64), 0, w.winsum, c.Sr, c.P.win, d_out_jac);
            return 0;
        });
    };
    if (QuadLane<F>::AVAILABLE && ctx->opt_msm_tail_quads && (size_t)c.Sr * c.P.B <= ((size_t)1 << 18)) return tail(QuadLane<F>());
    return tail(TailLane<F>());
}

template <class F>
int msm_batch_member(zkhip_ctx *ctx, const zkhip_bases *bases, size_t offset, size_t n, const uint32_t *d_scalars, uint32_t *slot, bool reuse_sort) {
    MsmCall c;
    ZK_TRY(msm_call_plan<F>(ctx, bases, offset, n, true, c, ctx->last_error));
    MsmBuffers<F> w(ctx, c);
    ZK_TRY(ws_place(ctx, w));
    if (c.P.S == 1) w.buckets = slot;
    ZK_TRY(msm_stages<F>(ctx, bases, c, w, d_scalars, reuse_sort));
    if (w.buckets != slot) ZK_HIP_CHECK(ctx, hipMemcpyAsync(slot, w.buckets, c.P.B * MsmBuffers<F>::PW * 4, hipMemcpyDeviceToDevice, ctx->stream));
    return 0;
}

struct BasesTmp {
    size_t words;
    uint32_t *tmp;
    template <class Arena>
    void layout(Arena &a) { a.take(tmp, words); }
};

template <class F>
int bases_precompute_t(zkhip_ctx *ctx, zkhip_bases *b) {
    constexpr int NL = FieldOps<F>::WORDS;
    if (!b->tables() || b->n == 0) return 0;
    const size_t chunk = 1u << 18;
    const int kept = b->local_windows() - (b->win_rank == 0 ? 1 : 0);
    if (kept <= 0) return 0;
    BasesTmp w = {(size_t)kept * 5 * NL * std::min(chunk, b->n), nullptr};
    ZK_TRY(ws_place(ctx, w));
    uint32_t *tmp = w.tmp;
    for (size_t lo = 0; lo < b->n; lo += chunk) {
        size_t cnt = std::min(chunk, b->n - lo);
        ZK_LAUNCH(ctx, "bases_precompute", bases_precompute_range<F>, grid_1d(cnt, 64), dim3(64), 0, b->d, (uint32_t)b->n,
                  (uint32_t)lo, (uint32_t)cnt, msm_make_windows(zk_scalar_bits(b->curve), b->ntab), (uint32_t)b->win_rank, (uint32_t)b->win_world, tmp);
    }
    return 0;
}

inline bool msm_same_entries(const zkhip_bases *a, size_t off_a, size_t n_a, const uint32_t *s_a, const zkhip_bases *b, size_t off_b, size_t n_b,
                             const uint32_t *s_b) {
    return s_a == s_b && n_a == n_b && off_a == off_b && a->curve == b->curve && a->n == b->n && a->c_tab == b->c_tab && a->ntab == b->ntab &&
           a->win_rank == b->win_rank && a->win_world == b->win_world && a->nslots == b->nslots && a->tables() && b->tables();
}

template <class F>
struct MsmBatchArea {
    static constexpr size_t PW = MsmBuffers<F>::PW;
    size_t count, slot_words, segsum_blocks;
    bool fold;
    uint32_t *slots, *segsum, *winsum, **d_ptrs;
    MsmFoldBuffers<F> fb;
    template <class Arena>
    void layout(Arena &a) {
        a.take(slots, count * slot_words);
        a.take(segsum, segsum_blocks * PW);
        a.take(winsum, count * PW);
        a.take(d_ptrs, count);
        if (fold) fb.layout(a);
    }
};

template <class F, class Lane>
int msm_batch_tail(zkhip_ctx *ctx, size_t count, const zkhip_bases *const *bases, const size_t *offsets, const size_t *ns,
                   const uint32_t *const *d_scalars, uint32_t *const *d_outs) {
    const uint32_t B = 1u << (bases[0]->c_tab - 1);
    size_t max_need = 0;
    for (size_t i = 0; i < count; ++i) {
        if (ns[i] == 0 || bases[i]->local_windows() == 0) continue;
        MsmCall c;
        ZK_TRY(msm_call_plan<F>(ctx, bases[i], offsets[i], ns[i], false, c, ctx->last_error));
        MsmBuffers<F> w(ctx, c);
        max_need = std::max(max_need, ws_bytes(w));
    }
    MsmBatchArea<F> area;
    area.count = count;
    area.slot_words = B * area.PW;
    area.segsum_blocks = count * msm_tail_geom<Lane>(ctx, B, count).nblk;
    area.fold = msm_fold_applies<F>(ctx, B, true);
    if (area.fold) area.fb = MsmFoldBuffers<F>(ctx, B, count);
    ctx->ws_floor = 0;
    ZK_TRY(ws_place(ctx, area, max_need));
    uint32_t *const slots = area.slots;
    const size_t slot_words = area.slot_words;
    uint32_t **d_ptrs = area.d_ptrs;
    ctx->ws_floor = ctx->ws_off;
    int rc = 0;
    size_t prev = (size_t)-1;
    for (size_t i = 0; i < count && rc == 0; ++i) {
        if (ns[i] == 0 || bases[i]->local_windows() == 0) {
            hipError_t e = hipMemsetAsync(slots + i * slot_words, 0, slot_words * 4, ctx->stream);
            if (e != hipSuccess) rc = ZKHIP_ERR_HIP;
        } else {
            const bool reuse = ctx->opt_msm_share_sort && prev != (size_t)-1 &&
                               msm_same_entries(bases[prev], offsets[prev], ns[prev], d_scalars[prev], bases[i], offsets[i], ns[i], d_scalars[i]);
            rc = msm_batch_member<F>(ctx, bases[i], offsets[i], ns[i], d_scalars[i], slots + i * slot_words, reuse);
            prev = i;
        }
    }
    ctx->ws_floor = 0;
    if (rc) return rc;
    if (ctx->batch_dptrs_override) {
        d_ptrs = static_cast<uint32_t **>(ctx->batch_dptrs_override);
    } else {
        ZK_TRY(ws_upload(ctx, d_ptrs, d_outs, count * sizeof(void *)));
    }
    if (area.fold) return msm_fold_tail<F, Lane>(ctx, slots, area.fb, d_ptrs, nullptr);
    return msm_tail<Lane>(ctx, slots, count, B, area.segsum, area.segsum_blocks, area.winsum, [&]() -> int {
        ZK_LAUNCH(ctx, "msm_final", (msm_final_batch<typename Lane::type, Lane::LANES>), dim3((unsigned)count), dim3(64), 0, area.winsum, (uint32_t)count, d_ptrs);
        return 0;
    });
}

template <class F>
int msm_batch_t(zkhip_ctx *ctx, size_t count, const zkhip_bases *const *bases, const size_t *offsets, const size_t *ns,
                const uint32_t *const *d_scalars, uint32_t *const *d_outs) {
    const size_t buckets = count << (bases[0]->c_tab - 1);
    if (!std::is_same<typename BucketLane<F>::type, typename TailLane<F>::type>::value && buckets >= ((size_t)1 << 21))
        return msm_batch_tail<F, BucketLane<F>>(ctx, count, bases, offsets, ns, d_scalars, d_outs);
    return msm_batch_tail<F, TailLane<F>>(ctx, count, bases, offsets, ns, d_scalars, d_outs);
}

template <class F>
int op_to_mont(zkhip_ctx *ctx, zkhip_bases *b, const uint32_t *d_canonical, const uint8_t *d_inf) {
    ZK_LAUNCH(ctx, "bases_to_mont", bases_to_mont<F>, grid_1d(b->n), dim3(256), 0, d_canonical, d_inf, (uint32_t)b->n, b->d);
    return 0;
}
template <class F>
int op_from_mont(zkhip_ctx *ctx, const zkhip_bases *b, size_t offset, size_t n, uint32_t *d_out, uint8_t *d_inf) {
    const uint32_t *src = b->d + offset * b->stride_u32;
    ZK_LAUNCH(ctx, "bases_from_mont", bases_from_mont<F>, grid_1d(n), dim3(256), 0, src, (uint32_t)n, d_out, d_inf);
    return 0;
}
template <class F>
struct FixedMulBuffers {
    size_t n;
    uint32_t *tab, *tmp;
    template <class Arena>
    void layout(Arena &a) {
        a.take(tab, (size_t)FIXED_NW * FIXED_ROW * 2 * FieldOps<F>::WORDS);
        a.take(tmp, std::max<size_t>((size_t)FIXED_NW * FIXED_ROW, n) * 5 * FieldOps<F>::WORDS);
    }
};
template <class F>
int op_mul(zkhip_ctx *ctx, zkhip_bases *b, const uint32_t *d_base_canonical, const uint32_t *d_scalars) {
    if (b->n < 4096) {
        ZK_LAUNCH(ctx, "bases_mul", bases_mul<F>, grid_1d(b->n, 64), dim3(64), 0, b->d, d_base_canonical, d_scalars, (uint32_t)b->n);
        return 0;
    }
    FixedMulBuffers<F> w = {b->n, nullptr, nullptr};
    ZK_TRY(ws_place(ctx, w));
    uint32_t *tab = w.tab, *tmp = w.tmp;
    ZK_LAUNCH(ctx, "bases_mul", bases_fixed_table<F>, dim3(1), dim3(64), 0, d_base_canonical, tab, tmp);
    const size_t lanes = (b->n + FIXED_CHUNK - 1) / FIXED_CHUNK;
    ZK_LAUNCH(ctx, "bases_mul", bases_mul_fixed<F>, grid_1d(lanes, 64), dim3(64), 0, b->d, tab, d_scalars, (uint32_t)b->n, tmp);
    return 0;
}
template <class F>
int op_jac_to_affine(zkhip_ctx *ctx, const uint32_t *d_jac, uint32_t *d_aff, uint8_t *d_inf) {
    ZK_LAUNCH(ctx, "jac_to_affine", jac_to_affine_k<F>, dim3(1), dim3(64), 0, d_jac, d_aff, d_inf);
    return 0;
}
template <class F>
int op_jac_sum(zkhip_ctx *ctx, const uint32_t *d_pts, size_t count, uint32_t *d_out) {
    ZK_LAUNCH(ctx, "jac_sum", jac_sum_k<F>, dim3(1), dim3(64), 0, d_pts, (uint32_t)count, d_out);
    return 0;
}
template <class F>
int op_write_infinity(zkhip_ctx *ctx, uint32_t *d_out_jac) {
    ZK_LAUNCH(ctx, "msm_write_infinity", msm_write_infinity<F>, dim3(1), dim3(64), 0, d_out_jac);
    return 0;
}

template <class F>
const MsmOps *msm_make_ops() {
    static const MsmOps ops = {msm_run_t<F>,        msm_batch_t<F>,      bases_precompute_t<F>, op_to_mont<F>,        op_from_mont<F>, op_mul<F>,
                               op_jac_to_affine<F>, op_jac_sum<F>, op_write_infinity<F>, (size_t)2 * FieldOps<F>::WORDS};
    return &ops;
}

}
```

### crypto3-zk_amd/csrc/msm_recode.hpp

```cpp
#pragma once
#include "zk_defs.hpp"

namespace zkhip {

static constexpr uint32_t DIG_NONE = 0xFFFFFFFFu;

ZK_HD uint32_t scalar_bits(const uint32_t *s, int lo, int c) {
    int limb = lo >> 5, off = lo & 31;
    if (limb >= 8) return 0;
    uint64_t v = s[limb];
    if (limb + 1 < 8) v |= (uint64_t)s[limb + 1] << 32;
    return (uint32_t)(v >> off) & ((1u << c) - 1);
}

struct MsmWindows {
    int tb, W;
    uint8_t offs[64];
    ZK_HD int off(int w) const { return W < 64 ? (int)offs[w] : (int)(((long long)w * tb) / W); }
    ZK_HD int width(int w) const { return off(w + 1) - off(w); }
};
inline MsmWindows msm_make_windows(int tb, int W) {
    MsmWindows m;
    m.tb = tb;
    m.W = W;
    for (int w = 0; w < 64; ++w) m.offs[w] = (uint8_t)(w <= W ? ((long long)w * tb) / W : 0);
    return m;
}

ZK_HD uint32_t msm_recode(const uint32_t *s, int off, int width, uint32_t &carry) {
    const uint32_t B = 1u << (width - 1);
    uint32_t d = scalar_bits(s, off, width) + carry;
    uint32_t neg = 0;
    carry = 0;
    if (d > B) {
        d = (1u << width) - d;
        neg = d != 0 ? 1u : 0u;
        carry = 1;
    }
    return d == 0 ? DIG_NONE : ((d - 1) | (neg << 31));
}

template <class FR>
ZK_HD bool msm_fold_scalar(const uint32_t *s, uint32_t out[8]) {
    uint32_t v[8], t[8];
#pragma unroll
    for (int i = 0; i < 8; ++i) v[i] = s[i];
    for (int it = 0; it < 6; ++it) {
        uint64_t borrow = 0;
#pragma unroll
        for (int i = 0; i < 8; ++i) {
            uint64_t d = (uint64_t)v[i] - FR::mod(i) - borrow;
            t[i] = (uint32_t)d;
            borrow = (d >> 32) & 1;
        }
        if (borrow) break;
#pragma unroll
        for (int i = 0; i < 8; ++i) v[i] = t[i];
    }
    uint64_t borrow = 0;
#pragma unroll
    for (int i = 0; i < 8; ++i) {
        uint64_t d = (uint64_t)FR::mod(i) - v[i] - borrow;
        t[i] = (uint32_t)d;
        borrow = (d >> 32) & 1;
    }
    bool fold = false, decided = false;
#pragma unroll
    for (int i = 7; i >= 0; --i) {
        if (!decided && v[i] != t[i]) {
            fold = v[i] > t[i];
            decided = true;
        }
    }
#pragma unroll
    for (int i = 0; i < 8; ++i) out[i] = fold ? t[i] : v[i];
    return fold;
}

ZK_HD int msm_windows(int rbits, int c) { return (rbits + c - 1) / c; }


}
```

### crypto3-zk_amd/csrc/zkhip.hip

```cpp
#include <algorithm>
#include <cstdlib>

#include "ctx.hpp"
#include "field_consts.hpp"
#include "msm_recode.hpp"
#include "zk_defs.hpp"

using namespace zkhip;

static int check_device(zkhip_ctx *ctx) {
    ZK_ENTER(ctx);
    return 0;
}

struct DownloadBuffers {
    size_t n, words;
    uint32_t *xy;
    uint8_t *inf;
    template <class Arena>
    void layout(Arena &a) {
        a.take(xy, n * words);
        a.take(inf, n);
    }
};
struct ToAffineBuffers {
    size_t cw;
    uint32_t *jac, *aff;
    uint8_t *inf;
    template <class Arena>
    void layout(Arena &a) {
        a.take(jac, 3 * cw);
        a.take(aff, 2 * cw);
        a.take(inf, 16);
    }
};

extern "C" {

const char *zkhip_strerror(int status) {
    switch (status) {
        case ZKHIP_OK: return "ok";
        case ZKHIP_ERR_NO_DEVICE: return "no usable HIP device (zkhip has no CPU fallback)";
        case ZKHIP_ERR_INVALID: return "invalid argument";
        case ZKHIP_ERR_HIP: return "HIP runtime error (see zkhip_last_error)";
        case ZKHIP_ERR_OOM: return "out of device memory";
        case ZKHIP_ERR_RANGE: return "size or offset out of range";
        case ZKHIP_ERR_NOT_FOUND: return "search ended without a result";
        default: return "unknown status";
    }
}

static std::mutex g_alloc_mutex;
static std::unordered_map<void *, zkhip_ctx *> g_block_owner;
static std::unordered_set<zkhip_ctx *> g_contexts;

int zkhip_init(int device_id, zkhip_ctx **out) {
    if (!out) return ZKHIP_ERR_INVALID;
    *out = nullptr;
    int count = 0;
    if (hipGetDeviceCount(&count) != hipSuccess || count <= 0) return ZKHIP_ERR_NO_DEVICE;
    if (device_id < 0 || device_id >= count) return ZKHIP_ERR_INVALID;
    if (hipSetDevice(device_id) != hipSuccess) return ZKHIP_ERR_NO_DEVICE;
    std::unique_ptr<zkhip_ctx> ctx(new zkhip_ctx());
    ctx->device = device_id;
    if (hipStreamCreateWithFlags(&ctx->stream, hipStreamNonBlocking) != hipSuccess) return ZKHIP_ERR_HIP;
    ctx->own_stream.reset(ctx->stream);
    if (ctx->d_status.alloc(ctx.get(), 4) != 0 || hipMemset(ctx->d_status, 0, 4) != hipSuccess) return ZKHIP_ERR_OOM;
    {
        std::lock_guard<std::mutex> g(g_alloc_mutex);
        g_contexts.insert(ctx.get());
    }
    if (const char *env = getenv("ZKHIP_OPTIONS"))
        zk_options_parse(env, [&](const char *name, int64_t value) { (void)zkhip_set_option(ctx.get(), name, value); });
    *out = ctx.release();
    return ZKHIP_OK;
}

static void alloc_cache_flush(zkhip_ctx *ctx);

}

zkhip_ctx::~zkhip_ctx() {
    (void)hipSetDevice(device);
    (void)hipStreamSynchronize(stream);
    ntt_tables.clear();
    ntt_ext_tables.clear();
    dom_tables.clear();
    dom_ws.reset();
    prof.pending.clear();
    prof.pool.clear();
    zk_graphs_clear(this);
    order_event.reset();
    {
        std::lock_guard<std::mutex> g(g_alloc_mutex);
        std::lock_guard<std::mutex> lock(alloc_mutex);
        alloc_cache_flush(this);
        for (auto &e : alloc_live) g_block_owner.erase(e.first);
        alloc_live.clear();
        g_contexts.erase(this);
    }
    msm_host_buf.reset();
    ws.reset();
    d_status.reset();
    own_stream.reset();
}

extern "C" {

void zkhip_destroy(zkhip_ctx *ctx) {
    if (ctx) delete ctx;
}

int zkhip_device(const zkhip_ctx *ctx) { return ctx ? ctx->device : -1; }

int zkhip_stream_wait(zkhip_ctx *waiter, zkhip_ctx *signal) {
    if (!waiter || !signal || waiter->device != signal->device) return ZKHIP_ERR_INVALID;
    if (waiter == signal) return ZKHIP_OK;
    ZK_HIP_CHECK(waiter, hipSetDevice(waiter->device));
    if (!signal->order_event) ZK_HIP_CHECK(waiter, zk_event_create(signal->order_event, hipEventDisableTiming));
    ZK_HIP_CHECK(waiter, hipEventRecord(signal->order_event.get(), signal->stream));
    ZK_HIP_CHECK(waiter, hipStreamWaitEvent(waiter->stream, signal->order_event.get(), 0));
    return ZKHIP_OK;
}

const char *zkhip_last_error(const zkhip_ctx *ctx) { return ctx ? ctx->last_error.c_str() : ""; }

int zkhip_set_stream(zkhip_ctx *ctx, void *hip_stream) {
    if (!ctx) return ZKHIP_ERR_INVALID;
    ZK_TRY(check_device(ctx));
    ZK_HIP_CHECK(ctx, hipStreamSynchronize(ctx->stream));
    ctx->own_stream.reset();
    ctx->stream = reinterpret_cast<hipStream_t>(hip_stream);
    return ZKHIP_OK;
}

int zkhip_sync(zkhip_ctx *ctx) {
    if (!ctx) return ZKHIP_ERR_INVALID;
    ZK_TRY(check_device(ctx));
    ZK_HIP_CHECK(ctx, hipStreamSynchronize(ctx->stream));
    return ZKHIP_OK;
}

int zkhip_device_status(zkhip_ctx *ctx, uint32_t *flags) {
    if (!ctx) return ZKHIP_ERR_INVALID;
    ZK_TRY(check_device(ctx));
    uint32_t f = 0;
    ZK_HIP_CHECK(ctx, hipMemcpyAsync(&f, ctx->d_status, 4, hipMemcpyDeviceToHost, ctx->stream));
    ZK_HIP_CHECK(ctx, hipStreamSynchronize(ctx->stream));
    if (f) ZK_HIP_CHECK(ctx, hipMemsetAsync(ctx->d_status, 0, 4, ctx->stream));
    if (flags) *flags = f;
    if (f) {
        ctx->last_error = std::string("device status:") + ((f & ZK_STATUS_GATHER_RANGE) ? " gather index out of range;" : "") +
                          ((f & ZK_STATUS_MSM_PLAN_OVERFLOW) ? " MSM large-bucket plan overflow;" : "");
        return ZKHIP_ERR_RANGE;
    }
    return ZKHIP_OK;
}

int zkhip_set_option(zkhip_ctx *ctx, const char *name, int64_t value) {
    if (!ctx || !name) return ZKHIP_ERR_INVALID;
    const OptRow<zkhip_ctx> *row = zk_option_find<zkhip_ctx>(name);
    if (!row) return ZKHIP_ERR_INVALID;
    if (row->admit != OPT_CUSTOM) {
        zk_option_store(*ctx, *row, value);
    } else if (!row->member) {
        if (value < 0) return ZKHIP_ERR_RANGE;
        std::lock_guard<std::mutex> g(g_alloc_mutex);
        std::lock_guard<std::mutex> lock(ctx->alloc_mutex);
        ctx->opt_alloc_cache_bytes = (size_t)value << 20;
        if (ctx->alloc_cached_bytes > ctx->opt_alloc_cache_bytes) alloc_cache_flush(ctx);
    } else if (row->member == &zkhip_ctx::opt_msm_shard_world) {
        if (value < 1 || value > 64) return ZKHIP_ERR_RANGE;
        ctx->opt_msm_shard_world = (int)value;
        if (ctx->opt_msm_shard_rank >= ctx->opt_msm_shard_world) ctx->opt_msm_shard_rank = 0;
    } else if (row->member == &zkhip_ctx::opt_msm_shard_rank) {
        if (value < 0 || value >= ctx->opt_msm_shard_world) return ZKHIP_ERR_RANGE;
        ctx->opt_msm_shard_rank = (int)value;
    } else if (row->member == &zkhip_ctx::opt_stream_priority) {
        if (!ctx->own_stream) return ZKHIP_ERR_INVALID;
        ZK_ENTER(ctx);
        int least = 0, greatest = 0;
        ZK_HIP_CHECK(ctx, hipDeviceGetStreamPriorityRange(&least, &greatest));
        ZK_HIP_CHECK(ctx, hipStreamSynchronize(ctx->stream));
        hipStream_t s = nullptr;
        ZK_HIP_CHECK(ctx, hipStreamCreateWithPriority(&s, hipStreamNonBlocking, value < 0 ? greatest : (value > 0 ? least : 0)));
        ctx->own_stream.reset(s);
        ctx->stream = s;
        ctx->opt_stream_priority = (int)value;
        zk_graphs_clear(ctx);
    } else {
        return ZKHIP_ERR_INVALID;
    }
    return ZKHIP_OK;
}

int zkhip_get_option(const zkhip_ctx *ctx, const char *name, int64_t *value) {
    if (!ctx || !name || !value) return ZKHIP_ERR_INVALID;
    const OptRow<zkhip_ctx> *row = zk_option_find<zkhip_ctx>(name);
    if (!row) return ZKHIP_ERR_INVALID;
    *value = row->member ? ctx->*row->member : (int64_t)(ctx->opt_alloc_cache_bytes >> 20);
    return ZKHIP_OK;
}

static void alloc_cache_flush(zkhip_ctx *ctx) {
    for (auto &e : ctx->alloc_free) {
        g_block_owner.erase(e.second);
        (void)hipFree(e.second);
    }
    ctx->alloc_free.clear();
    ctx->alloc_cached_bytes = 0;
}
int zkhip_malloc(zkhip_ctx *ctx, size_t bytes, void **dptr) {
    if (!ctx || !dptr) return ZKHIP_ERR_INVALID;
    ZK_TRY(check_device(ctx));
    const size_t want = ((bytes ? bytes : 1) + 0xFFFF) & ~(size_t)0xFFFF;
    {
        std::lock_guard<std::mutex> lock(ctx->alloc_mutex);
        auto it = ctx->alloc_free.lower_bound(want);
        if (it != ctx->alloc_free.end() && it->first <= want + (want >> 3)) {
            *dptr = it->second;
            ctx->alloc_cached_bytes -= it->first;
            ctx->alloc_live[*dptr] = it->first;
            ctx->alloc_free.erase(it);
            return ZKHIP_OK;
        }
    }
    hipError_t e = hipMalloc(dptr, want);
    if (e != hipSuccess) {
        (void)hipGetLastError();
        std::lock_guard<std::mutex> g(g_alloc_mutex);
        for (zkhip_ctx *c : g_contexts)
            if (c->device == ctx->device) {
                std::lock_guard<std::mutex> lock(c->alloc_mutex);
                alloc_cache_flush(c);
            }
        e = hipMalloc(dptr, want);
    }
    ZK_HIP_CHECK(ctx, e);
    std::lock_guard<std::mutex> g(g_alloc_mutex);
    std::lock_guard<std::mutex> lock(ctx->alloc_mutex);
    ctx->alloc_live[*dptr] = want;
    g_block_owner[*dptr] = ctx;
    return ZKHIP_OK;
}
int zkhip_free(zkhip_ctx *ctx, void *dptr) {
    if (!ctx) return ZKHIP_ERR_INVALID;
    if (!dptr) return ZKHIP_OK;
    int block_device = ctx->device;
    {
        std::lock_guard<std::mutex> g(g_alloc_mutex);
        auto own = g_block_owner.find(dptr);
        if (own != g_block_owner.end()) block_device = own->second->device;
    }
    ZK_HIP_CHECK(ctx, hipSetDevice(block_device));
    ZK_HIP_CHECK(ctx, hipDeviceSynchronize());
    std::lock_guard<std::mutex> g(g_alloc_mutex);
    auto own = g_block_owner.find(dptr);
    if (own == g_block_owner.end()) {
        ZK_HIP_CHECK(ctx, hipFree(dptr));
        return ZKHIP_OK;
    }
    zkhip_ctx *owner = own->second;
    std::lock_guard<std::mutex> lock(owner->alloc_mutex);
    auto it = owner->alloc_live.find(dptr);
    if (it == owner->alloc_live.end()) return ZKHIP_ERR_INVALID;
    const size_t sz = it->second;
    owner->alloc_live.erase(it);
    if (sz <= owner->opt_alloc_cache_bytes && owner->alloc_cached_bytes + sz <= owner->opt_alloc_cache_bytes) {
        owner->alloc_free.emplace(sz, dptr);
        owner->alloc_cached_bytes += sz;
        return ZKHIP_OK;
    }
    g_block_owner.erase(own);
    ZK_HIP_CHECK(ctx, hipFree(dptr));
    return ZKHIP_OK;
}
int zkhip_memcpy_h2d(zkhip_ctx *ctx, void *dst, const void *src, size_t bytes) {
    if (!ctx) return ZKHIP_ERR_INVALID;
    ZK_TRY(check_device(ctx));
    ZK_HIP_CHECK(ctx, hipMemcpyAsync(dst, src, bytes, hipMemcpyHostToDevice, ctx->stream));
    ZK_HIP_CHECK(ctx, hipStreamSynchronize(ctx->stream));
    return ZKHIP_OK;
}
int zkhip_memcpy_h2d_async(zkhip_ctx *ctx, void *dst, const void *src, size_t bytes) {
    if (!ctx) return ZKHIP_ERR_INVALID;
    ZK_TRY(check_device(ctx));
    ZK_HIP_CHECK(ctx, hipMemcpyAsync(dst, src, bytes, hipMemcpyHostToDevice, ctx->stream));
    return ZKHIP_OK;
}
int zkhip_host_alloc(zkhip_ctx *ctx, size_t bytes, void **hptr) {
    if (!ctx || !hptr) return ZKHIP_ERR_INVALID;
    ZK_ENTER(ctx);
    ZK_HIP_CHECK(ctx, hipHostMalloc(hptr, bytes ? bytes : 1, hipHostMallocPortable));
    return ZKHIP_OK;
}
int zkhip_host_free(zkhip_ctx *ctx, void *hptr) {
    if (!ctx) return ZKHIP_ERR_INVALID;
    ZK_TRY(check_device(ctx));
    ZK_HIP_CHECK(ctx, hipStreamSynchronize(ctx->stream));
    ZK_HIP_CHECK(ctx, hipHostFree(hptr));
    return ZKHIP_OK;
}
int zkhip_memcpy_d2h(zkhip_ctx *ctx, void *dst, const void *src, size_t bytes) {
    if (!ctx) return ZKHIP_ERR_INVALID;
    ZK_TRY(check_device(ctx));
    ZK_HIP_CHECK(ctx, hipMemcpyAsync(dst, src, bytes, hipMemcpyDeviceToHost, ctx->stream));
    ZK_HIP_CHECK(ctx, hipStreamSynchronize(ctx->stream));
    return ZKHIP_OK;
}

int zkhip_memcpy_d2h_async(zkhip_ctx *ctx, void *dst, const void *src, size_t bytes) {
    if (!ctx) return ZKHIP_ERR_INVALID;
    ZK_TRY(check_device(ctx));
    ZK_HIP_CHECK(ctx, hipMemcpyAsync(dst, src, bytes, hipMemcpyDeviceToHost, ctx->stream));
    return ZKHIP_OK;
}

int zkhip_memcpy_d2d_async(zkhip_ctx *ctx, void *dst, const void *src, size_t bytes) {
    if (!ctx) return ZKHIP_ERR_INVALID;
    ZK_TRY(check_device(ctx));
    ZK_HIP_CHECK(ctx, hipMemcpyAsync(dst, src, bytes, hipMemcpyDeviceToDevice, ctx->stream));
    return ZKHIP_OK;
}

int zkhip_memcpy_2d_d2d_async(zkhip_ctx *ctx, void *dst, size_t dst_pitch, const void *src, size_t src_pitch, size_t width, size_t rows) {
    if (!ctx) return ZKHIP_ERR_INVALID;
    if (width == 0 || rows == 0) return ZKHIP_OK;
    if (!dst || !src || width > dst_pitch || width > src_pitch) return ZKHIP_ERR_INVALID;
    ZK_TRY(check_device(ctx));
    if (dst_pitch >= ((size_t)1 << 31) || src_pitch >= ((size_t)1 << 31)) {
        for (size_t r = 0; r < rows; ++r)
            ZK_HIP_CHECK(ctx, hipMemcpyAsync(static_cast<char *>(dst) + r * dst_pitch, static_cast<const char *>(src) + r * src_pitch, width, hipMemcpyDeviceToDevice,
                                             ctx->stream));
        return ZKHIP_OK;
    }
    ZK_HIP_CHECK(ctx, hipMemcpy2DAsync(dst, dst_pitch, src, src_pitch, width, rows, hipMemcpyDeviceToDevice, ctx->stream));
    return ZKHIP_OK;
}

static int bases_alloc(zkhip_ctx *ctx, int curve, int group, size_t n, std::unique_ptr<zkhip_bases> &out) {
    if (!zk_curve_group_known(curve, group)) return ZKHIP_ERR_INVALID;
    std::unique_ptr<zkhip_bases> b(new zkhip_bases());
    b->curve = curve;
    b->group = group;
    b->n = n;
    b->stride_u32 = zk_point_words(curve, group);
    const bool shard = ctx->opt_msm_shard_world > 1;
    if (ctx->opt_msm_precompute && n >= (size_t)ctx->opt_msm_precompute_min) {
        b->c_tab = ctx->opt_msm_window_bits > 0 ? std::max(2, std::min(ZK_MSM_MAX_C, ctx->opt_msm_window_bits)) : zk_msm_auto_window(n);
        b->ntab = msm_windows(zk_scalar_bits(curve), b->c_tab);
        if (shard) {
            b->win_rank = ctx->opt_msm_shard_rank;
            b->win_world = ctx->opt_msm_shard_world;
        }
        b->nslots = shard ? b->local_windows() + (b->win_rank != 0 ? 1 : 0) : b->ntab;
        if (b->nslots < 1) b->nslots = 1;
    } else if (shard) {
        b->win_rank = ctx->opt_msm_shard_rank;
        b->win_world = ctx->opt_msm_shard_world;
    }
    int rc = b->d.alloc(ctx, std::max<size_t>(1, n) * b->nslots * b->stride_u32 * 4);
    if (rc && b->tables() && !shard) {
        b->ntab = 1;
        b->c_tab = 0;
        b->nslots = 1;
        rc = b->d.alloc(ctx, std::max<size_t>(1, n) * b->stride_u32 * 4);
    }
    ZK_TRY(rc);
    out = std::move(b);
    return 0;
}

static int bases_finish(zkhip_ctx *ctx, std::unique_ptr<zkhip_bases> &b, zkhip_bases **out) {
    ZK_TRY(zk_bases_precompute(ctx, b.get()));
    ZK_HIP_CHECK(ctx, hipStreamSynchronize(ctx->stream));
    *out = b.release();
    return ZKHIP_OK;
}

}

template <class P>
static bool coords_canonical(const uint64_t *xy, const uint8_t *inf, size_t n) {
    uint64_t m[4];
    for (int i = 0; i < 4; ++i) m[i] = (uint64_t)P::mod(2 * i) | ((uint64_t)P::mod(2 * i + 1) << 32);
    for (size_t i = 0; i < n; ++i) {
        if (inf && inf[i]) continue;
        for (int k = 0; k < 2; ++k) {
            const uint64_t *c = xy + (2 * i + k) * 4;
            int j = 3;
            while (j > 0 && c[j] == m[j]) --j;
            if (c[j] >= m[j]) return false;
        }
    }
    return true;
}

extern "C" {

int zkhip_bases_upload(zkhip_ctx *ctx, int curve, int group, const uint64_t *affine_xy, const uint8_t *is_infinity, size_t n,
                       zkhip_bases **out) {
    if (!ctx || !out || (n && !affine_xy)) return ZKHIP_ERR_INVALID;
    if (group == GROUP_G1 && ((curve == CURVE_PALLAS && !coords_canonical<PallasFq>(affine_xy, is_infinity, n)) ||
                              (curve == CURVE_VESTA && !coords_canonical<VestaFq>(affine_xy, is_infinity, n)))) {
        ctx->last_error = "zkhip_bases_upload: a coordinate is not below the base-field modulus";
        return ZKHIP_ERR_INVALID;
    }
    ZK_TRY(check_device(ctx));
    std::unique_ptr<zkhip_bases> b;
    ZK_TRY(bases_alloc(ctx, curve, group, n, b));
    DevBuf d_canon, d_inf;
    if (n) {
        const size_t cbytes = n * 2 * zk_coord_limbs64(curve, group) * 8;
        ZK_TRY(d_canon.alloc(ctx, cbytes));
        ZK_HIP_CHECK(ctx, hipMemcpyAsync(d_canon, affine_xy, cbytes, hipMemcpyHostToDevice, ctx->stream));
        if (is_infinity) {
            ZK_TRY(d_inf.alloc(ctx, n));
            ZK_HIP_CHECK(ctx, hipMemcpyAsync(d_inf, is_infinity, n, hipMemcpyHostToDevice, ctx->stream));
        }
        ZK_TRY(zk_bases_to_mont(ctx, b.get(), d_canon, d_inf.as<uint8_t>()));
    }
    return bases_finish(ctx, b, out);
}

int zkhip_bases_upload_compressed(zkhip_ctx *ctx, int curve, int group, const uint8_t *octets, size_t n, zkhip_bases **out) {
    ZK_ARGS_PAIRING(ctx, curve);
    if (!out || (n && !octets)) return ZKHIP_ERR_INVALID;
    if (curve != CURVE_BLS12_381) return ZKHIP_ERR_INVALID;
    ZK_TRY(check_device(ctx));
    std::unique_ptr<zkhip_bases> b;
    ZK_TRY(bases_alloc(ctx, curve, group, n, b));
    DevBuf d_oct;
    if (n) {
        const size_t bytes = n * (group == GROUP_G2 ? 96 : 48);
        ZK_TRY(d_oct.alloc(ctx, bytes + 16));
        uint32_t *d_err = reinterpret_cast<uint32_t *>(d_oct.as<uint8_t>() + ((bytes + 3) & ~(size_t)3));
        ZK_HIP_CHECK(ctx, hipMemcpyAsync(d_oct, octets, bytes, hipMemcpyHostToDevice, ctx->stream));
        ZK_HIP_CHECK(ctx, hipMemsetAsync(d_err, 0, 4, ctx->stream));
        ZK_TRY(zk_bases_decompress(ctx, b.get(), d_oct.as<uint8_t>(), d_err));
        uint32_t rejected = 0;
        ZK_HIP_CHECK(ctx, hipMemcpyAsync(&rejected, d_err, 4, hipMemcpyDeviceToHost, ctx->stream));
        ZK_HIP_CHECK(ctx, hipStreamSynchronize(ctx->stream));
        if (rejected) {
            ctx->last_error = std::to_string(rejected) + " point encoding(s) rejected (flags, x >= p, or x not on the curve)";
            return ZKHIP_ERR_INVALID;
        }
    }
    return bases_finish(ctx, b, out);
}

static const uint64_t GEN_BLS_G1[12] = {0xfb3af00adb22c6bbULL, 0x6c55e83ff97a1aefULL, 0xa14e3a3f171bac58ULL, 0xc3688c4f9774b905ULL,
                                        0x2695638c4fa9ac0fULL, 0x17f1d3a73197d794ULL, 0x0caa232946c5e7e1ULL, 0xd03cc744a2888ae4ULL,
                                        0x00db18cb2c04b3edULL, 0xfcf5e095d5d00af6ULL, 0xa09e30ed741d8ae4ULL, 0x08b3f481e3aaa0f1ULL};
static const uint64_t GEN_BLS_G2[24] = {
    0xd48056c8c121bdb8ULL, 0x0bac0326a805bbefULL, 0xb4510b647ae3d177ULL, 0xc6e47ad4fa403b02ULL, 0x260805272dc51051ULL, 0x024aa2b2f08f0a91ULL,
    0xe5ac7d055d042b7eULL, 0x334cf11213945d57ULL, 0xb5da61bbdc7f5049ULL, 0x596bd0d09920b61aULL, 0x7dacd3a088274f65ULL, 0x13e02b6052719f60ULL,
    0xe193548608b82801ULL, 0x923ac9cc3baca289ULL, 0x6d429a695160d12cULL, 0xadfd9baa8cbdd3a7ULL, 0x8cc9cdc6da2e351aULL, 0x0ce5d527727d6e11ULL,
    0xaaa9075ff05f79beULL, 0x3f370d275cec1da1ULL, 0x267492ab572e99abULL, 0xcb3e287e85a763afULL, 0x32acd2b02bc28b99ULL, 0x0606c4a02ea734ccULL};
static const uint64_t GEN_BN_G1[8] = {1, 0, 0, 0, 2, 0, 0, 0};
static const uint64_t GEN_PALLAS_G1[8] = {0x992d30ed00000000ULL, 0x224698fc094cf91bULL, 0, 0x4000000000000000ULL, 2, 0, 0, 0};
static const uint64_t GEN_VESTA_G1[8] = {0x8c46eb2100000000ULL, 0x224698fc0994a8ddULL, 0, 0x4000000000000000ULL, 2, 0, 0, 0};
static const uint64_t GEN_BN_G2[16] = {0x46debd5cd992f6edULL, 0x674322d4f75edaddULL, 0x426a00665e5c4479ULL, 0x1800deef121f1e76ULL,
                                       0x97e485b7aef312c2ULL, 0xf1aa493335a9e712ULL, 0x7260bfb731fb5d25ULL, 0x198e9393920d483aULL,
                                       0x4ce6cc0166fa7daaULL, 0xe3d1e7690c43d37bULL, 0x4aab71808dcb408fULL, 0x12c85ea5db8c6debULL,
                                       0x55acdadcd122975bULL, 0xbc4b313370b38ef3ULL, 0xec9e99ad690c3395ULL, 0x090689d0585ff075ULL};

int zkhip_bases_from_scalars(zkhip_ctx *ctx, int curve, int group, const uint64_t *base_affine_xy, const uint64_t *scalars, size_t n,
                             zkhip_bases **out) {
    if (!ctx || !out || (n && !scalars)) return ZKHIP_ERR_INVALID;
    ZK_TRY(check_device(ctx));
    std::unique_ptr<zkhip_bases> b;
    ZK_TRY(bases_alloc(ctx, curve, group, n, b));
    const uint64_t *gen = base_affine_xy;
    if (!gen)
        gen = curve == CURVE_PALLAS  ? GEN_PALLAS_G1
              : curve == CURVE_VESTA ? GEN_VESTA_G1
              : curve == CURVE_BLS12_381 ? (group == GROUP_G1 ? GEN_BLS_G1 : GEN_BLS_G2)
                                         : (group == GROUP_G1 ? GEN_BN_G1 : GEN_BN_G2);
    DevBuf d_s, d_g;
    if (n) {
        const size_t gbytes = 2 * zk_coord_limbs64(curve, group) * 8;
        ZK_TRY(d_s.alloc(ctx, n * 32));
        ZK_TRY(d_g.alloc(ctx, gbytes));
        ZK_HIP_CHECK(ctx, hipMemcpyAsync(d_s, scalars, n * 32, hipMemcpyHostToDevice, ctx->stream));
        ZK_HIP_CHECK(ctx, hipMemcpyAsync(d_g, gen, gbytes, hipMemcpyHostToDevice, ctx->stream));
        ZK_TRY(zk_bases_mul(ctx, b.get(), d_g, d_s));
    }
    return bases_finish(ctx, b, out);
}

__global__ void bases_spread_rows(const uint32_t *__restrict__ src, size_t count, uint32_t stride, const uint32_t *__restrict__ d_rows, uint32_t first,
                                  uint32_t n_total, uint32_t *__restrict__ out, uint32_t *__restrict__ status) {
    const size_t g = (size_t)blockIdx.x * blockDim.x + threadIdx.x;
    if (g >= count * stride) return;
    const size_t j = g / stride;
    const uint32_t w = (uint32_t)(g % stride), row = d_rows ? d_rows[j] : first + (uint32_t)j;
    if (row >= n_total || (d_rows && j + 1 < count && d_rows[j + 1] <= row)) {
        if (w == 0) atomicOr(status, ZK_STATUS_GATHER_RANGE);
        if (row >= n_total) return;
    }
    out[(size_t)row * stride + w] = src[g];
}

int zkhip_bases_spread(zkhip_ctx *ctx, const zkhip_bases *src, const uint32_t *d_rows, size_t first, size_t n_total, zkhip_bases **out) {
    if (!ctx || !src || !out) return ZKHIP_ERR_INVALID;
    if (n_total >= ((size_t)1 << 32) || (!d_rows && first + src->n > n_total)) return ZKHIP_ERR_RANGE;
    if (src->n * src->stride_u32 >= ((size_t)1 << 39)) return ZKHIP_ERR_RANGE;
    ZK_TRY(check_device(ctx));
    std::unique_ptr<zkhip_bases> b;
    ZK_TRY(bases_alloc(ctx, src->curve, src->group, n_total, b));
    if (n_total) {
        ZK_HIP_CHECK(ctx, hipMemsetAsync(b->d, 0, n_total * b->stride_u32 * 4, ctx->stream));
        if (src->n) {
            const size_t lanes = src->n * src->stride_u32;
            ZK_LAUNCH(ctx, "bases_spread_rows", bases_spread_rows, grid_1d(lanes), dim3(256), 0, src->d, src->n,
                      (uint32_t)src->stride_u32, d_rows, (uint32_t)first, (uint32_t)n_total, b->d, ctx->d_status);
        }
    }
    return bases_finish(ctx, b, out);
}

int zkhip_bases_download(zkhip_ctx *ctx, const zkhip_bases *b, size_t offset, size_t n, uint64_t *affine_xy, uint8_t *is_infinity) {
    if (!ctx || !b || (n && (!affine_xy || !is_infinity))) return ZKHIP_ERR_INVALID;
    if (offset + n > b->n) return ZKHIP_ERR_RANGE;
    if (n == 0) return ZKHIP_OK;
    ZK_TRY(check_device(ctx));
    size_t pbytes = n * 2 * zk_coord_limbs64(b->curve, b->group) * 8;
    DownloadBuffers w = {n, 4 * zk_coord_limbs64(b->curve, b->group)};
    ZK_TRY(ws_place(ctx, w));
    uint32_t *d_out = w.xy;
    uint8_t *d_inf = w.inf;
    ZK_TRY(zk_bases_from_mont(ctx, b, offset, n, d_out, d_inf));
    ZK_HIP_CHECK(ctx, hipMemcpyAsync(affine_xy, d_out, pbytes, hipMemcpyDeviceToHost, ctx->stream));
    ZK_HIP_CHECK(ctx, hipMemcpyAsync(is_infinity, d_inf, n, hipMemcpyDeviceToHost, ctx->stream));
    ZK_HIP_CHECK(ctx, hipStreamSynchronize(ctx->stream));
    return ZKHIP_OK;
}

size_t zkhip_bases_size(const zkhip_bases *b) { return b ? b->n : 0; }

void zkhip_bases_free(zkhip_ctx *ctx, zkhip_bases *b) {
    if (!b) return;
    if (ctx) {
        (void)hipSetDevice(ctx->device);
        (void)hipStreamSynchronize(ctx->stream);
    }
    delete b;
}

int zkhip_msm_dev(zkhip_ctx *ctx, const zkhip_bases *bases, size_t offset, size_t n, const void *d_scalars, void *d_out_jacobian) {
    if (!ctx || !bases || !d_out_jacobian || (n && !d_scalars)) return ZKHIP_ERR_INVALID;
    ZK_TRY(check_device(ctx));
    return zk_msm_run(ctx, bases, offset, n, (const uint32_t *)d_scalars, (uint32_t *)d_out_jacobian);
}

int zkhip_msm_batch_dev(zkhip_ctx *ctx, size_t count, const zkhip_bases *const *bases, const size_t *offsets, const size_t *ns,
                        const void *const *d_scalars, void *const *d_out_jacobian) {
    if (!ctx || (count && (!bases || !offsets || !ns || !d_scalars || !d_out_jacobian))) return ZKHIP_ERR_INVALID;
    for (size_t i = 0; i < count; ++i)
        if (!bases[i] || !d_out_jacobian[i] || (ns[i] && !d_scalars[i])) return ZKHIP_ERR_INVALID;
    ZK_TRY(check_device(ctx));
    return zk_msm_run_batch(ctx, count, bases, offsets, ns, (const uint32_t *const *)d_scalars, (uint32_t *const *)d_out_jacobian);
}

}

int zk_msm_host_reserve(zkhip_ctx *ctx, size_t n) {
    const size_t want = std::max<size_t>(1, n) * 32 + 512;
    if (ctx->msm_host_buf.cap >= want) return 0;
    ZK_HIP_CHECK(ctx, hipStreamSynchronize(ctx->stream));
    zk_graphs_clear(ctx);
    return ctx->msm_host_buf.reserve(ctx, want);
}

extern "C" {

int zkhip_msm(zkhip_ctx *ctx, const zkhip_bases *bases, size_t offset, size_t n, const uint64_t *scalars, uint64_t *out_jacobian) {
    if (!ctx || !bases || !out_jacobian || (n && !scalars)) return ZKHIP_ERR_INVALID;
    ZK_TRY(check_device(ctx));
    const size_t obytes = 3 * zk_coord_limbs64(bases->curve, bases->group) * 8;
    ZK_TRY(zk_msm_host_reserve(ctx, n));
    uint32_t *d_o = ctx->msm_host_buf.as<uint32_t>(), *d_s = d_o + 128;
    if (n) ZK_HIP_CHECK(ctx, hipMemcpyAsync(d_s, scalars, n * 32, hipMemcpyHostToDevice, ctx->stream));
    ZK_TRY(zk_msm_run(ctx, bases, offset, n, d_s, d_o));
    ZK_HIP_CHECK(ctx, hipMemcpyAsync(out_jacobian, d_o, obytes, hipMemcpyDeviceToHost, ctx->stream));
    ZK_HIP_CHECK(ctx, hipStreamSynchronize(ctx->stream));
    return ZKHIP_OK;
}

int zkhip_jacobian_sum_dev(zkhip_ctx *ctx, int curve, int group, const void *d_points, size_t count, void *d_out_jacobian) {
    if (!ctx || !d_points || !d_out_jacobian) return ZKHIP_ERR_INVALID;
    if (!zk_curve_group_known(curve, group)) return ZKHIP_ERR_INVALID;
    ZK_TRY(check_device(ctx));
    return zk_jac_sum(ctx, curve, group, (const uint32_t *)d_points, count, (uint32_t *)d_out_jacobian);
}

int zkhip_jacobian_to_affine(zkhip_ctx *ctx, int curve, int group, const uint64_t *jacobian, uint64_t *affine_xy, uint8_t *is_infinity) {
    if (!ctx || !jacobian || !affine_xy || !is_infinity) return ZKHIP_ERR_INVALID;
    if (!zk_curve_group_known(curve, group)) return ZKHIP_ERR_INVALID;
    ZK_TRY(check_device(ctx));
    size_t cl = zk_coord_limbs64(curve, group) * 8;
    ToAffineBuffers w = {cl / 4};
    ZK_TRY(ws_place(ctx, w));
    uint32_t *d_j = w.jac, *d_a = w.aff;
    uint8_t *d_i = w.inf;
    ZK_HIP_CHECK(ctx, hipMemcpyAsync(d_j, jacobian, 3 * cl, hipMemcpyHostToDevice, ctx->stream));
    ZK_TRY(zk_jac_to_affine(ctx, curve, group, d_j, d_a, d_i));
    ZK_HIP_CHECK(ctx, hipMemcpyAsync(affine_xy, d_a, 2 * cl, hipMemcpyDeviceToHost, ctx->stream));
    ZK_HIP_CHECK(ctx, hipMemcpyAsync(is_infinity, d_i, 1, hipMemcpyDeviceToHost, ctx->stream));
    ZK_HIP_CHECK(ctx, hipStreamSynchronize(ctx->stream));
    return ZKHIP_OK;
}

int zkhip_ntt_dev(zkhip_ctx *ctx, int curve, void *d_data, size_t log_m, size_t batch, const uint64_t *omega, int inverse,
                  const uint64_t *coset_gen) {
    if (!ctx || !omega || (batch && !d_data)) return ZKHIP_ERR_INVALID;
    ZK_TRY(check_device(ctx));
    return zk_ntt_run(ctx, curve, (uint32_t *)d_data, log_m, batch, omega, inverse ? 1 : 0, coset_gen);
}

int zkhip_ntt(zkhip_ctx *ctx, int curve, uint64_t *data, size_t log_m, size_t batch, const uint64_t *omega, int inverse,
              const uint64_t *coset_gen) {
    if (!ctx || !omega || (batch && !data)) return ZKHIP_ERR_INVALID;
    if (log_m > 32) return ZKHIP_ERR_RANGE;
    if (batch == 0) return ZKHIP_OK;
    ZK_TRY(check_device(ctx));
    size_t bytes = (batch << log_m) * 32;
    DevBuf d;
    ZK_TRY(d.alloc(ctx, bytes));
    ZK_HIP_CHECK(ctx, hipMemcpyAsync(d, data, bytes, hipMemcpyHostToDevice, ctx->stream));
    ZK_TRY(zk_ntt_run(ctx, curve, d, log_m, batch, omega, inverse ? 1 : 0, coset_gen));
    ZK_HIP_CHECK(ctx, hipMemcpyAsync(data, d, bytes, hipMemcpyDeviceToHost, ctx->stream));
    ZK_HIP_CHECK(ctx, hipStreamSynchronize(ctx->stream));
    return ZKHIP_OK;
}

int zkhip_profile_enable(zkhip_ctx *ctx, int on) {
    if (!ctx) return ZKHIP_ERR_INVALID;
    ctx->prof_collect();
    ctx->prof.on = on != 0;
    return ZKHIP_OK;
}
int zkhip_profile_filter(zkhip_ctx *ctx, const char *prefix) {
    if (!ctx) return ZKHIP_ERR_INVALID;
    ctx->prof_collect();
    ctx->prof.filter = prefix ? prefix : "";
    return ZKHIP_OK;
}
int zkhip_profile_reset(zkhip_ctx *ctx) {
    if (!ctx) return ZKHIP_ERR_INVALID;
    ctx->prof_collect();
    ctx->prof.acc.clear();
    return ZKHIP_OK;
}
int zkhip_profile_get(zkhip_ctx *ctx, const char *prefix, double *total_ms, uint64_t *launches) {
    if (!ctx || !prefix) return ZKHIP_ERR_INVALID;
    ctx->prof_collect();
    double ms = 0;
    uint64_t cnt = 0;
    size_t pl = strlen(prefix);
    for (auto &kv : ctx->prof.acc) {
        if (kv.first.compare(0, pl, prefix) == 0) {
            ms += kv.second.first;
            cnt += kv.second.second;
        }
    }
    if (total_ms) *total_ms = ms;
    if (launches) *launches = cnt;
    return ZKHIP_OK;
}
size_t zkhip_profile_dump(zkhip_ctx *ctx, char *buf, size_t cap) {
    if (!ctx) return 0;
    ctx->prof_collect();
    std::string s;
    char line[256];
    for (auto &kv : ctx->prof.acc) {
        snprintf(line, sizeof(line), "%s %.6f %llu\n", kv.first.c_str(), kv.second.first, (unsigned long long)kv.second.second);
        s += line;
    }
    if (buf && cap) {
        size_t k = std::min(cap - 1, s.size());
        memcpy(buf, s.data(), k);
        buf[k] = 0;
    }
    return s.size() + 1;
}

}
```

Before: 397.4 Mpoints/s.

## Fuse scalar recoding into sort kernels and fold size histogram and large plan

Drops the separate digit-recoding kernel and its digit buffer. The sort histogram and split kernels now recode scalars on the fly per point and emit entries for every window, tiling by points, with the tile point count chosen so the tile count is a multiple of the CU count. The split kernel reuses the histogram counts instead of recounting. The size histogram moves into sort_final, large-bucket planning merges into size_scatter, and the level2 memset is replaced by in-kernel zeroing. The cost is recomputing the recode twice per point, in histogram and split, in exchange for fewer launches and less global traffic.

```diff
diff --git a/__graft_entry__.py b/__graft_entry__.py
--- a/__graft_entry__.py
+++ b/__graft_entry__.py
@@ -27,6 +27,7 @@
     subprocess.check_call(["make", "-C", os.path.join(ROOT, "tests", "cpp"), "-f", "pow.mk"], env=env)
     subprocess.check_call(["make", "-j2", "-C", os.path.join(ROOT, "tests", "cpp"), "-f", "pasta.mk"], env=env)
     subprocess.check_call(["make", "-C", os.path.join(ROOT, "tests", "cpp"), "-f", "ipa.mk"], env=env)
+    subprocess.check_call(["make", "-C", os.path.join(ROOT, "tests", "cpp"), "-f", "msm_sort.mk"], env=env)
     zk = _load_pkg()
     zk.load_library()
 
diff --git a/crypto3-zk_amd/csrc/ctx.hpp b/crypto3-zk_amd/csrc/ctx.hpp
--- a/crypto3-zk_amd/csrc/ctx.hpp
+++ b/crypto3-zk_amd/csrc/ctx.hpp
@@ -187,6 +187,7 @@
 
 struct zkhip_ctx {
     int device = 0;
+    int cu_count = 0;
     hipStream_t stream = nullptr;
     StreamOwner own_stream;
     EventOwner order_event;
diff --git a/crypto3-zk_amd/csrc/hosttest.hip b/crypto3-zk_amd/csrc/hosttest.hip
--- a/crypto3-zk_amd/csrc/hosttest.hip
+++ b/crypto3-zk_amd/csrc/hosttest.hip
@@ -101,6 +101,8 @@
     return W;
 }
 
+uint32_t zkt_msm_sort_tile_points(uint64_t n, uint32_t W, uint32_t tile, uint32_t cus) { return msm_sort_tile_points((size_t)n, W, tile, cus); }
+
 int zkt_sha256_elements(const uint64_t *elems, size_t n, uint8_t *digest) {
     if (!elems || !digest || n == 0) return -1;
     sha256::hash_elements(elems, n, digest);
diff --git a/crypto3-zk_amd/csrc/msm_core.hpp b/crypto3-zk_amd/csrc/msm_core.hpp
--- a/crypto3-zk_amd/csrc/msm_core.hpp
+++ b/crypto3-zk_amd/csrc/msm_core.hpp
@@ -132,37 +132,6 @@
     return 0;
 }
 
-template <class FR>
-__global__ __launch_bounds__(256) void msm_digits_only(const uint32_t *__restrict__ scalars, uint32_t n, MsmWindows win, uint32_t wrank,
-                                                       uint32_t wworld, uint32_t *__restrict__ dig) {
-    uint32_t i = blockIdx.x * blockDim.x + threadIdx.x;
-    if (i >= n) return;
-    uint32_t s[8];
-    const uint32_t flip = msm_fold_scalar<FR>(scalars + (size_t)i * 8, s) ? 0x80000000u : 0u;
-    uint32_t carry = 0, next = wrank, lw = 0;
-    for (int w = 0; w < win.W; ++w) {
-        uint32_t d = msm_recode(s, win.off(w), win.width(w), carry);
-        if ((uint32_t)w != next) continue;
-        dig[(size_t)lw * n + i] = d == DIG_NONE ? d : d ^ flip;
-        next += wworld;
-        ++lw;
-    }
-}
-
-struct SortGeom {
-    uint32_t n;
-    uint32_t W;
-    uint32_t B;
-    uint32_t S;
-    uint32_t lowb;
-    uint32_t nsuper;
-    uint32_t tile;
-    uint32_t ntile;
-    uint32_t slot0;
-    uint32_t tables;
-    uint32_t bases_n;
-    uint32_t base_off;
-};
 struct SortBig {
     static constexpr uint32_t TILE = 16384, THREADS = 1024;
 };
@@ -172,26 +141,18 @@
 constexpr uint32_t SORT_MAX_LOW = 10;
 constexpr uint32_t SORT_MAX_SUPER = 1024;
 
-ZK_D uint32_t sort_key(const SortGeom &g, uint32_t w, uint32_t d) { return (w % g.S) * g.B + (d & 0x7FFFFFFFu); }
-ZK_D uint32_t sort_entry(const SortGeom &g, uint32_t w, uint32_t i, uint32_t d) {
-    return ((g.tables ? (g.slot0 + w) * g.bases_n : 0u) + g.base_off + i) | (d & 0x80000000u);
-}
-
-template <class SZ>
-__global__ __launch_bounds__(SZ::THREADS) void msm_sort_hist(const uint32_t *__restrict__ dig, SortGeom g, uint32_t *__restrict__ bh) {
-    constexpr uint32_t SORT_TILE = SZ::TILE, SORT_THREADS = SZ::THREADS;
+template <class SZ, class FR>
+__global__ __launch_bounds__(SZ::THREADS) void msm_sort_hist(const uint32_t *__restrict__ scalars, SortGeom g, MsmWindows win, uint32_t *__restrict__ bh) {
+    constexpr uint32_t SORT_THREADS = SZ::THREADS;
     extern __shared__ uint32_t lh[];
-    const uint32_t tile = blockIdx.x, w = blockIdx.y, t = threadIdx.x;
+    const uint32_t tile = blockIdx.x, t = threadIdx.x;
     for (uint32_t k = t; k < g.nsuper; k += SORT_THREADS) lh[k] = 0;
     __syncthreads();
-    const uint32_t lo = tile * SORT_TILE, hi = min(g.n, lo + SORT_TILE);
-    for (uint32_t i = lo + t; i < hi; i += SORT_THREADS) {
-        uint32_t d = dig[(size_t)w * g.n + i];
-        if (d != DIG_NONE) atomicAdd(&lh[sort_key(g, w, d) >> g.lowb], 1u);
-    }
-    __syncthreads();
-    const size_t col = (size_t)w * g.ntile + tile, stride = (size_t)g.W * g.ntile;
-    for (uint32_t k = t; k < g.nsuper; k += SORT_THREADS) bh[(size_t)k * stride + col] = lh[k];
+    const uint32_t lo = tile * g.pts, hi = min(g.n, lo + g.pts);
+    for (uint32_t i = lo + t; i < hi; i += SORT_THREADS)
+        msm_point_entries<FR>(scalars + (size_t)i * 8, win, g, i, [&](uint32_t key, uint32_t) { atomicAdd(&lh[key >> g.lowb], 1u); });
+    __syncthreads();
+    for (uint32_t k = t; k < g.nsuper; k += SORT_THREADS) bh[(size_t)k * g.ntile + tile] = lh[k];
 }
 
 template <uint32_t SORT_THREADS>
@@ -213,9 +174,10 @@
     return total;
 }
 
-template <class SZ>
-__global__ __launch_bounds__(SZ::THREADS) void msm_sort_split(const uint32_t *__restrict__ dig, SortGeom g, const uint32_t *__restrict__ bo,
-                                                              uint32_t *__restrict__ tmp_idx, uint16_t *__restrict__ tmp_key) {
+template <class SZ, class FR>
+__global__ __launch_bounds__(SZ::THREADS) void msm_sort_split(const uint32_t *__restrict__ scalars, SortGeom g, MsmWindows win,
+                                                              const uint32_t *__restrict__ bo, uint32_t *__restrict__ tmp_idx,
+                                                              uint16_t *__restrict__ tmp_key) {
     constexpr uint32_t SORT_TILE = SZ::TILE, SORT_THREADS = SZ::THREADS;
     extern __shared__ uint32_t sm[];
     uint32_t *loff = sm;
@@ -224,31 +186,24 @@
     uint32_t *scratch = gbase + g.nsuper;
     uint32_t *sidx = scratch + SORT_THREADS;
     uint32_t *skey = sidx + SORT_TILE;
-    const uint32_t tile = blockIdx.x, w = blockIdx.y, t = threadIdx.x;
-    const size_t col = (size_t)w * g.ntile + tile, stride = (size_t)g.W * g.ntile;
+    const uint32_t tile = blockIdx.x, t = threadIdx.x;
     for (uint32_t k = t; k < g.nsuper; k += SORT_THREADS) {
-        loff[k] = 0;
-        gbase[k] = bo[(size_t)k * stride + col];
-    }
-    __syncthreads();
-    const uint32_t lo = tile * SORT_TILE, hi = min(g.n, lo + SORT_TILE);
-    for (uint32_t i = lo + t; i < hi; i += SORT_THREADS) {
-        uint32_t d = dig[(size_t)w * g.n + i];
-        if (d != DIG_NONE) atomicAdd(&loff[sort_key(g, w, d) >> g.lowb], 1u);
-    }
-    __syncthreads();
+        const uint32_t *b = bo + (size_t)k * g.ntile + tile;
+        gbase[k] = b[0];
+        loff[k] = b[1] - b[0];
+    }
+    __syncthreads();
+    const uint32_t lo = tile * g.pts, hi = min(g.n, lo + g.pts);
     const uint32_t total = block_excl_scan<SORT_THREADS>(loff, g.nsuper, scratch);
     if (t == 0) loff[g.nsuper] = total;
     for (uint32_t k = t; k < g.nsuper; k += SORT_THREADS) cur[k] = loff[k];
     __syncthreads();
-    for (uint32_t i = lo + t; i < hi; i += SORT_THREADS) {
-        uint32_t d = dig[(size_t)w * g.n + i];
-        if (d == DIG_NONE) continue;
-        const uint32_t key = sort_key(g, w, d);
-        const uint32_t r = atomicAdd(&cur[key >> g.lowb], 1u);
-        sidx[r] = sort_entry(g, w, i, d);
-        skey[r] = key;
-    }
+    for (uint32_t i = lo + t; i < hi; i += SORT_THREADS)
+        msm_point_entries<FR>(scalars + (size_t)i * 8, win, g, i, [&](uint32_t key, uint32_t entry) {
+            const uint32_t r = atomicAdd(&cur[key >> g.lowb], 1u);
+            sidx[r] = entry;
+            skey[r] = key;
+        });
     __syncthreads();
     const uint32_t lmask = (1u << g.lowb) - 1;
     for (uint32_t s = t; s < total; s += SORT_THREADS) {
@@ -256,6 +211,13 @@
         tmp_idx[pos] = sidx[s];
         tmp_key[pos] = (uint16_t)(key & lmask);
     }
+}
+
+constexpr uint32_t SIZE_BINS = MSM_LARGE_BUCKET + 2;
+
+ZK_D uint32_t size_bin(uint32_t size, uint32_t large) {
+    if (size == 0 || size > large) return SIZE_BINS - 1;
+    return size > MSM_LARGE_BUCKET ? 0 : 1 + MSM_LARGE_BUCKET - size;
 }
 
 constexpr uint32_t SORT_NLOW_MAX = 1u << SORT_MAX_LOW;
@@ -281,18 +243,20 @@
 template <class SZ>
 __global__ __launch_bounds__(SZ::THREADS) void msm_sort_final(const uint32_t *__restrict__ tmp_idx, const uint16_t *__restrict__ tmp_key, SortGeom g,
                                                               uint32_t nb, const uint32_t *__restrict__ bo, uint32_t *__restrict__ offs,
-                                                              uint32_t *__restrict__ idx) {
+                                                              uint32_t *__restrict__ idx, uint32_t large, uint32_t *__restrict__ sh,
+                                                              uint32_t *__restrict__ plan) {
     constexpr uint32_t SORT_TILE = SZ::TILE, SORT_THREADS = SZ::THREADS;
-    __shared__ uint32_t cnt[SORT_NLOW_MAX], cursor[SORT_NLOW_MAX], loff[SORT_NLOW_MAX], cur[SORT_NLOW_MAX], scratch[SORT_THREADS];
+    __shared__ uint32_t cnt[SORT_NLOW_MAX], cursor[SORT_NLOW_MAX], loff[SORT_NLOW_MAX], cur[SORT_NLOW_MAX], scratch[SORT_THREADS], sbin[SIZE_BINS];
     extern __shared__ uint32_t sm[];
     uint32_t *sidx = sm;
     uint16_t *skey = reinterpret_cast<uint16_t *>(sidx + SORT_TILE);
     const uint32_t grp = blockIdx.x, t = threadIdx.x;
-    const size_t stride = (size_t)g.W * g.ntile;
-    const uint32_t start = bo[(size_t)grp * stride];
-    const uint32_t end = bo[(size_t)(grp + 1) * stride];
+    const uint32_t start = bo[(size_t)grp * g.ntile];
+    const uint32_t end = bo[(size_t)(grp + 1) * g.ntile];
     const uint32_t nlow = 1u << g.lowb;
+    if (grp == 0 && t < 4) plan[t] = 0;
     for (uint32_t k = t; k < SORT_NLOW_MAX; k += SORT_THREADS) cnt[k] = 0;
+    for (uint32_t k = t; k < SIZE_BINS; k += SORT_THREADS) sbin[k] = 0;
     __syncthreads();
     for (uint32_t k = start + t; k < end; k += SORT_THREADS) atomicAdd(&cnt[tmp_key[k]], 1u);
     __syncthreads();
@@ -300,10 +264,14 @@
     for (uint32_t k = t; k < nlow; k += SORT_THREADS) {
         const uint32_t bucket = grp * nlow + k;
         cursor[k] += start;
-        if (bucket < nb) offs[bucket] = cursor[k];
+        if (bucket < nb) {
+            offs[bucket] = cursor[k];
+            atomicAdd(&sbin[size_bin(cnt[k], large)], 1u);
+        }
     }
     if (grp + 1 == g.nsuper && t == 0) offs[nb] = end;
     __syncthreads();
+    for (uint32_t k = t; k < SIZE_BINS; k += SORT_THREADS) sh[(size_t)k * g.nsuper + grp] = sbin[k];
     for (uint32_t c0 = start; c0 < end; c0 += SORT_TILE) {
         const uint32_t c1 = min(end, c0 + SORT_TILE);
         for (uint32_t k = t; k < SORT_NLOW_MAX; k += SORT_THREADS) cnt[k] = 0;
@@ -330,57 +298,41 @@
     }
 }
 
-constexpr uint32_t SIZE_BINS = MSM_LARGE_BUCKET + 2;
-
-ZK_D uint32_t size_bin(uint32_t size, uint32_t large) {
-    if (size == 0 || size > large) return SIZE_BINS - 1;
-    return size > MSM_LARGE_BUCKET ? 0 : 1 + MSM_LARGE_BUCKET - size;
-}
-
-__global__ __launch_bounds__(256) void msm_size_hist(const uint32_t *__restrict__ offs, uint32_t nbuckets, uint32_t nblocks,
-                                                     uint32_t large, uint32_t *__restrict__ bh) {
-    __shared__ uint32_t lh[SIZE_BINS];
-    const uint32_t t = threadIdx.x;
-    if (t < SIZE_BINS) lh[t] = 0;
-    __syncthreads();
-    for (uint32_t g = blockIdx.x * 1024 + t; g < min(nbuckets, (blockIdx.x + 1) * 1024); g += 256)
-        atomicAdd(&lh[size_bin(offs[g + 1] - offs[g], large)], 1u);
-    __syncthreads();
-    if (t < SIZE_BINS) bh[(size_t)t * nblocks + blockIdx.x] = lh[t];
-}
-
-__global__ __launch_bounds__(256) void msm_size_scatter(const uint32_t *__restrict__ offs, uint32_t nbuckets, uint32_t nblocks,
-                                                        uint32_t large, const uint32_t *__restrict__ bo, uint32_t *__restrict__ order) {
+struct LargePlan {
+    uint32_t *plan, *tasks, *large;
+    uint32_t task_cap, large_cap;
+    uint32_t *status;
+};
+ZK_D void msm_plan_bucket(const LargePlan &p, uint32_t g, uint32_t lo, uint32_t hi) {
+    const uint32_t nt = (hi - lo + MSM_LARGE_CHUNK - 1) / MSM_LARGE_CHUNK;
+    const uint32_t first = atomicAdd(&p.plan[0], nt);
+    const uint32_t slot = atomicAdd(&p.plan[1], 1u);
+    if (first + nt > p.task_cap || slot >= p.large_cap) {
+        atomicOr(p.status, ZK_STATUS_MSM_PLAN_OVERFLOW);
+        return;
+    }
+    for (uint32_t t = 0; t < nt; ++t) {
+        p.tasks[3 * (first + t)] = g;
+        p.tasks[3 * (first + t) + 1] = lo + t * MSM_LARGE_CHUNK;
+        p.tasks[3 * (first + t) + 2] = min(hi, lo + (t + 1) * MSM_LARGE_CHUNK);
+    }
+    p.large[3 * slot] = g;
+    p.large[3 * slot + 1] = first;
+    p.large[3 * slot + 2] = nt;
+}
+
+__global__ __launch_bounds__(256) void msm_size_scatter(const uint32_t *__restrict__ offs, uint32_t nbuckets, uint32_t lowb, uint32_t nblocks,
+                                                        uint32_t large, const uint32_t *__restrict__ bo, uint32_t *__restrict__ order, LargePlan lp) {
     __shared__ uint32_t cur[SIZE_BINS];
     const uint32_t t = threadIdx.x;
     if (t < SIZE_BINS) cur[t] = bo[(size_t)t * nblocks + blockIdx.x];
     __syncthreads();
-    for (uint32_t g = blockIdx.x * 1024 + t; g < min(nbuckets, (blockIdx.x + 1) * 1024); g += 256)
-        order[atomicAdd(&cur[size_bin(offs[g + 1] - offs[g], large)], 1u)] = g;
-}
-
-__global__ __launch_bounds__(256) void msm_plan_large(const uint32_t *__restrict__ offs, uint32_t nbuckets, uint32_t *__restrict__ plan,
-                                                      uint32_t *__restrict__ tasks, uint32_t *__restrict__ large, uint32_t task_cap,
-                                                      uint32_t large_cap, uint32_t thresh, uint32_t *__restrict__ status) {
-    uint32_t g = blockIdx.x * blockDim.x + threadIdx.x;
-    if (g >= nbuckets) return;
-    uint32_t lo = offs[g], hi = offs[g + 1], size = hi - lo;
-    if (size <= thresh) return;
-    uint32_t nt = (size + MSM_LARGE_CHUNK - 1) / MSM_LARGE_CHUNK;
-    uint32_t first = atomicAdd(&plan[0], nt);
-    uint32_t slot = atomicAdd(&plan[1], 1u);
-    if (first + nt > task_cap || slot >= large_cap) {
-        atomicOr(status, ZK_STATUS_MSM_PLAN_OVERFLOW);
-        return;
-    }
-    for (uint32_t t = 0; t < nt; ++t) {
-        tasks[3 * (first + t)] = g;
-        tasks[3 * (first + t) + 1] = lo + t * MSM_LARGE_CHUNK;
-        tasks[3 * (first + t) + 2] = min(hi, lo + (t + 1) * MSM_LARGE_CHUNK);
-    }
-    large[3 * slot] = g;
-    large[3 * slot + 1] = first;
-    large[3 * slot + 2] = nt;
+    const uint32_t first = blockIdx.x << lowb, last = min(nbuckets, first + (1u << lowb));
+    for (uint32_t g = first + t; g < last; g += 256) {
+        const uint32_t lo = offs[g], hi = offs[g + 1];
+        order[atomicAdd(&cur[size_bin(hi - lo, large)], 1u)] = g;
+        if (hi - lo > large) msm_plan_bucket(lp, g, lo, hi);
+    }
 }
 
 template <class F, int LPB>
@@ -570,6 +522,10 @@
         if (col || o != 0)
             xyzz_store<FT>(level2 + (((size_t)2 * w + (col ? 0 : 1)) * g.C + (col ? o : o - 1)) * PW, xyzz_load<FT>(lds + (size_t)i * m * PW));
     }
+    if (!col && wg == 0) {
+        uint32_t *empty = level2 + ((size_t)2 * w + 1) * g.C * PW;
+        for (uint32_t k = (g.R - 1) * PW + threadIdx.x; k < g.C * PW; k += MSM_TAIL_THREADS) empty[k] = 0;
+    }
 }
 
 template <class F>
@@ -891,7 +847,6 @@
     constexpr int QL = QuadLane<F>::LANES;
     const MsmFold &g = fb.g;
     const size_t nsets = fb.nsets;
-    ZK_HIP_CHECK(ctx, hipMemsetAsync(fb.level2, 0, fb.level2_words() * 4, ctx->stream));
     const size_t lds = (size_t)MSM_TAIL_THREADS / LPB * 4 * NL * 4;
     ZK_MAX_LDS(ctx, (msm_fold<FL, LPB, TQ, QL>), lds);
     ZK_LAUNCH(ctx, "msm_fold", (msm_fold<FL, LPB, TQ, QL>), dim3((unsigned)(nsets * (g.B / (MSM_TAIL_THREADS / LPB * g.run)) * 2)), dim3(MSM_TAIL_THREADS), lds,
@@ -939,18 +894,18 @@
     return p;
 }
 
-template <class SZ>
-int msm_sort_run(zkhip_ctx *ctx, const SortGeom &g, uint32_t nbh, const uint32_t *dig, uint32_t *bh, uint32_t *bo, uint32_t *bsums, uint32_t *tmp_idx,
-                 uint16_t *tmp_key, uint32_t *offs, uint32_t *idx) {
+template <class SZ, class FR>
+int msm_sort_run(zkhip_ctx *ctx, const SortGeom &g, const MsmWindows &win, uint32_t nbh, const uint32_t *d_scalars, uint32_t *bh, uint32_t *bo, uint32_t *bsums,
+                 uint32_t *tmp_idx, uint16_t *tmp_key, uint32_t *offs, uint32_t *idx, uint32_t large, uint32_t *sh, uint32_t *plan) {
     const size_t lds_hist = (size_t)g.nsuper * 4;
     const size_t lds_split = ((size_t)3 * g.nsuper + 1 + SZ::THREADS + 2 * SZ::TILE) * 4;
     const size_t lds_final = (size_t)SZ::TILE * 6;
-    if (lds_split > 48 * 1024) ZK_MAX_LDS(ctx, msm_sort_split<SZ>, 160 * 1024 - 256);
-    if (lds_final > 40 * 1024) ZK_MAX_LDS(ctx, msm_sort_final<SZ>, 160 * 1024 - (4 * SORT_NLOW_MAX + SZ::THREADS) * 4 - 256);
-    ZK_LAUNCH(ctx, "msm_sort_hist", msm_sort_hist<SZ>, dim3(g.ntile, g.W), dim3(SZ::THREADS), lds_hist, dig, g, bh);
+    if (lds_split > 48 * 1024) ZK_MAX_LDS(ctx, (msm_sort_split<SZ, FR>), 160 * 1024 - 256);
+    if (lds_final > 40 * 1024) ZK_MAX_LDS(ctx, msm_sort_final<SZ>, 160 * 1024 - (4 * SORT_NLOW_MAX + SZ::THREADS + SIZE_BINS) * 4 - 256);
+    ZK_LAUNCH(ctx, "msm_sort_hist", (msm_sort_hist<SZ, FR>), dim3(g.ntile), dim3(SZ::THREADS), lds_hist, d_scalars, g, win, bh);
     ZK_TRY(msm_scan(ctx, "msm_scan", bh, nbh, bo, bsums));
-    ZK_LAUNCH(ctx, "msm_sort_split", msm_sort_split<SZ>, dim3(g.ntile, g.W), dim3(SZ::THREADS), lds_split, dig, g, bo, tmp_idx, tmp_key);
-    ZK_LAUNCH(ctx, "msm_sort_final", msm_sort_final<SZ>, dim3(g.nsuper), dim3(SZ::THREADS), lds_final, tmp_idx, tmp_key, g, g.S * g.B, bo, offs, idx);
+    ZK_LAUNCH(ctx, "msm_sort_split", (msm_sort_split<SZ, FR>), dim3(g.ntile), dim3(SZ::THREADS), lds_split, d_scalars, g, win, bo, tmp_idx, tmp_key);
+    ZK_LAUNCH(ctx, "msm_sort_final", msm_sort_final<SZ>, dim3(g.nsuper), dim3(SZ::THREADS), lds_final, tmp_idx, tmp_key, g, g.S * g.B, bo, offs, idx, large, sh, plan);
     return 0;
 }
 
@@ -959,7 +914,7 @@
     SortGeom g;
     bool big_tiles;
     uint32_t nbh;
-    uint32_t sblk, nsh;
+    uint32_t nsh;
     int Sr;
     uint32_t segsum_blocks;
     bool fold;
@@ -983,17 +938,19 @@
     g.nsuper = (P.nb + (1u << g.lowb) - 1) >> g.lowb;
     c.big_tiles = ctx->opt_msm_sort_tile_log >= 14;
     g.tile = c.big_tiles ? SortBig::TILE : SortSmall::TILE;
-    g.ntile = (uint32_t)((n + g.tile - 1) / g.tile);
+    g.pts = msm_sort_tile_points(n, g.W, g.tile, (uint32_t)std::max(0, ctx->cu_count));
+    g.ntile = (uint32_t)((n + g.pts - 1) / g.pts);
+    g.wrank = P.wrank;
+    g.wworld = P.wworld;
     g.tables = P.tables ? 1u : 0u;
     g.slot0 = P.tables ? (uint32_t)bases->slot_of_local(0) : 0u;
     g.bases_n = (uint32_t)bases->n;
     g.base_off = (uint32_t)offset;
-    if (g.nsuper > SORT_MAX_SUPER) return ZKHIP_ERR_RANGE;
-    const size_t nbh64 = (size_t)g.nsuper * g.W * g.ntile;
+    if (g.nsuper > SORT_MAX_SUPER || (uint64_t)g.pts * g.W > g.tile) return ZKHIP_ERR_RANGE;
+    const size_t nbh64 = (size_t)g.nsuper * g.ntile;
     if (nbh64 >= (1ull << 31)) return ZKHIP_ERR_RANGE;
     c.nbh = (uint32_t)nbh64;
-    c.sblk = (P.nb + 1023) / 1024;
-    c.nsh = SIZE_BINS * c.sblk;
+    c.nsh = SIZE_BINS * g.nsuper;
     c.Sr = P.tables ? 1 : P.W;
     c.segsum_blocks = std::max(msm_tail_geom<TailLane<F>>(ctx, P.B, c.Sr).nblk, msm_tail_geom<QuadLane<F>>(ctx, P.B, c.Sr).nblk);
     c.fold = !batch_member && msm_fold_applies<F>(ctx, P.B, P.tables);
@@ -1007,7 +964,7 @@
 struct MsmBuffers {
     static constexpr size_t PW = (size_t)4 * FieldOps<F>::WORDS;
     const MsmCall &c;
-    uint32_t *dig, *bh, *bo, *bsums, *tmp_idx;
+    uint32_t *bh, *bo, *bsums, *tmp_idx;
     uint16_t *tmp_key;
     uint32_t *offs, *idx, *buckets;
     uint32_t *sh, *so, *ssums, *order;
@@ -1019,7 +976,6 @@
     }
     template <class Arena>
     void layout(Arena &a) {
-        a.take(dig, c.entries());
         a.take(bh, c.nbh);
         a.take(bo, (size_t)c.nbh + 1);
         a.take(bsums, (c.nbh + 1023) / 1024);
@@ -1048,18 +1004,17 @@
     typedef typename BucketLane<F>::type FL;
     constexpr int LPB = BucketLane<F>::LANES;
     const MsmPlan &P = c.P;
-    const uint32_t n = c.g.n, nb = P.nb;
+    const uint32_t nb = P.nb;
     const uint32_t *d_b = bases->d;
     if (!reuse_sort) {
         ZK_TRY(fr_sat_dispatch(bases->curve, [&](auto fr) -> int {
             typedef typename decltype(fr)::type FR;
-            ZK_LAUNCH(ctx, "msm_digits", msm_digits_only<FR>, grid_1d(n), dim3(256), 0, d_scalars, n, P.win, P.wrank, P.wworld, w.dig);
-            return 0;
+            return (c.big_tiles ? msm_sort_run<SortBig, FR> : msm_sort_run<SortSmall, FR>)(ctx, c.g, P.win, c.nbh, d_scalars, w.bh, w.bo, w.bsums, w.tmp_idx, w.tmp_key,
+                                                                                             w.offs, w.idx, c.large_thresh, w.sh, w.plan);
         }));
-        ZK_TRY((c.big_tiles ? msm_sort_run<SortBig> : msm_sort_run<SortSmall>)(ctx, c.g, c.nbh, w.dig, w.bh, w.bo, w.bsums, w.tmp_idx, w.tmp_key, w.offs, w.idx));
-        ZK_LAUNCH(ctx, "msm_size_sort", msm_size_hist, dim3(c.sblk), dim3(256), 0, w.offs, nb, c.sblk, c.large_thresh, w.sh);
         ZK_TRY(msm_scan(ctx, "msm_size_sort", w.sh, c.nsh, w.so, w.ssums));
-        ZK_LAUNCH(ctx, "msm_size_sort", msm_size_scatter, dim3(c.sblk), dim3(256), 0, w.offs, nb, c.sblk, c.large_thresh, w.so, w.order);
+        const LargePlan lp = {w.plan, w.tasks, w.large, c.task_cap, c.large_cap, ctx->d_status};
+        ZK_LAUNCH(ctx, "msm_size_sort", msm_size_scatter, dim3(c.g.nsuper), dim3(256), 0, w.offs, nb, c.g.lowb, c.g.nsuper, c.large_thresh, w.so, w.order, lp);
     }
     if constexpr (FieldOps<F>::WORDS <= 16) {
         constexpr int NT = MSM_G1_THREADS;
@@ -1073,11 +1028,6 @@
         ZK_MAX_LDS(ctx, (msm_bucket_acc_lds<FL, NT, WAVES, LPB>), lds_acc);
         ZK_LAUNCH(ctx, "msm_bucket_acc", (msm_bucket_acc_lds<FL, NT, WAVES, LPB>), dim3((unsigned)(((size_t)nb * LPB + NT - 1) / NT)), dim3(NT), lds_acc, d_b,
                   w.offs, w.idx, nb, c.large_thresh, w.order, w.buckets);
-    }
-    if (!reuse_sort) {
-        ZK_HIP_CHECK(ctx, hipMemsetAsync(w.plan, 0, 16, ctx->stream));
-        ZK_LAUNCH(ctx, "msm_plan_large", msm_plan_large, grid_1d(nb), dim3(256), 0, w.offs, nb, w.plan, w.tasks, w.large, c.task_cap, c.large_cap,
-                  c.large_thresh, ctx->d_status);
     }
     {
         size_t lds_large = (size_t)128 / LPB * 4 * NL * 4;
diff --git a/crypto3-zk_amd/csrc/msm_recode.hpp b/crypto3-zk_amd/csrc/msm_recode.hpp
--- a/crypto3-zk_amd/csrc/msm_recode.hpp
+++ b/crypto3-zk_amd/csrc/msm_recode.hpp
@@ -79,5 +79,78 @@
 
 ZK_HD int msm_windows(int rbits, int c) { return (rbits + c - 1) / c; }
 
+struct SortGeom {
+    uint32_t n;
+    uint32_t W;
+    uint32_t B;
+    uint32_t S;
+    uint32_t lowb;
+    uint32_t nsuper;
+    uint32_t tile;
+    uint32_t pts;
+    uint32_t ntile;
+    uint32_t slot0;
+    uint32_t tables;
+    uint32_t bases_n;
+    uint32_t base_off;
+    uint32_t wrank, wworld;
+};
+
+ZK_HD uint32_t sort_key(const SortGeom &g, uint32_t w, uint32_t d) { return (w % g.S) * g.B + (d & 0x7FFFFFFFu); }
+ZK_HD uint32_t sort_entry(const SortGeom &g, uint32_t w, uint32_t i, uint32_t d) {
+    return ((g.tables ? (g.slot0 + w) * g.bases_n : 0u) + g.base_off + i) | (d & 0x80000000u);
+}
+
+ZK_HD uint32_t msm_recode_word(uint64_t v, uint32_t sh, uint32_t width, uint32_t &carry) {
+    const uint32_t B = 1u << (width - 1);
+    uint32_t d = ((uint32_t)(v >> sh) & ((1u << width) - 1)) + carry;
+    uint32_t neg = 0;
+    carry = 0;
+    if (d > B) {
+        d = (1u << width) - d;
+        neg = d != 0 ? 1u : 0u;
+        carry = 1;
+    }
+    return d == 0 ? DIG_NONE : ((d - 1) | (neg << 31));
+}
+
+template <class FR, class Emit>
+ZK_HD void msm_point_entries(const uint32_t *scalar, const MsmWindows &win, const SortGeom &g, uint32_t i, Emit &&emit) {
+    uint32_t s[8];
+    const uint32_t flip = msm_fold_scalar<FR>(scalar, s) ? 0x80000000u : 0u;
+    const uint32_t W = (uint32_t)win.W, q = (uint32_t)win.tb / W, rem = (uint32_t)win.tb % W;
+    uint32_t carry = 0, next = g.wrank, lw = 0, w = 0, off = 0, err = 0;
+    ZK_UNROLL
+    for (uint32_t limb = 0; limb < 8; ++limb) {
+        const uint64_t v = (uint64_t)s[limb] | (limb + 1 < 8 ? (uint64_t)s[limb + 1] << 32 : 0);
+        while (w < W && (off >> 5) == limb) {
+            uint32_t width = q;
+            err += rem;
+            if (err >= W) {
+                err -= W;
+                ++width;
+            }
+            const uint32_t d = msm_recode_word(v, off & 31, width, carry);
+            off += width;
+            if (w++ != next) continue;
+            if (d != DIG_NONE) emit(sort_key(g, lw, d ^ flip), sort_entry(g, lw, i, d ^ flip));
+            next += g.wworld;
+            ++lw;
+        }
+    }
+}
+
+inline uint32_t msm_sort_tile_points(size_t n, uint32_t W, uint32_t tile, uint32_t cus) {
+    if (W == 0) W = 1;
+    const uint32_t pmax = tile / W > 0 ? tile / W : 1u, pmin = tile / (2 * W) > 0 ? tile / (2 * W) : 1u;
+    if (cus > 1) {
+        for (uint32_t p = pmax; p >= pmin; --p) {
+            const size_t tiles = (n + p - 1) / p;
+            if (tiles > 0 && tiles % cus == 0) return (uint32_t)((n + tiles - 1) / tiles);
+        }
+    }
+    return pmax;
+}
+
 
 }
diff --git a/crypto3-zk_amd/csrc/zkhip.hip b/crypto3-zk_amd/csrc/zkhip.hip
--- a/crypto3-zk_amd/csrc/zkhip.hip
+++ b/crypto3-zk_amd/csrc/zkhip.hip
@@ -63,6 +63,7 @@
     if (hipSetDevice(device_id) != hipSuccess) return ZKHIP_ERR_NO_DEVICE;
     std::unique_ptr<zkhip_ctx> ctx(new zkhip_ctx());
     ctx->device = device_id;
+    if (hipDeviceGetAttribute(&ctx->cu_count, hipDeviceAttributeMultiprocessorCount, device_id) != hipSuccess) ctx->cu_count = 0;
     if (hipStreamCreateWithFlags(&ctx->stream, hipStreamNonBlocking) != hipSuccess) return ZKHIP_ERR_HIP;
     ctx->own_stream.reset(ctx->stream);
     if (ctx->d_status.alloc(ctx.get(), 4) != 0 || hipMemset(ctx->d_status, 0, 4) != hipSuccess) return ZKHIP_ERR_OOM;
```

Measured after the change: 404.9 Mpoints/s, median of 6. No clear change (+1.9%).
